# davidesantangelo/krep

Measured on NVIDIA H100. Metric: GB/s scanned (HBM-resident corpus), higher is better.
Workload: dtype u8

## Files before the change

### include/krep_b200.h

```cpp
#ifndef KREP_B200_H
#define KREP_B200_H

#include <stdbool.h>
#include <stddef.h>
#include <stdint.h>

#ifdef __cplusplus
extern "C" {
#endif

#ifndef KREP_H

typedef struct
{
   size_t start_offset;
   size_t end_offset;
} match_position_t;

typedef struct match_result_t
{
   match_position_t *positions;
   uint64_t count;
   uint64_t capacity;
} match_result_t;

struct ac_trie;
typedef struct ac_trie ac_trie_t;

typedef struct search_params
{
   const char *pattern;
   size_t pattern_len;

   const char **patterns;
   size_t *pattern_lens;
   size_t num_patterns;

   bool case_sensitive;
   bool use_regex;
   bool count_lines_mode;
   bool count_matches_mode;
   bool track_positions;
   bool whole_word;

   const void *compiled_regex;
   ac_trie_t *ac_trie;
   size_t max_count;
} search_params_t;

typedef uint64_t (*search_func_t)(const search_params_t *params,
                                  const char *text_start,
                                  size_t text_len,
                                  match_result_t *result);
#endif


int krep_b200_init(int device);
int krep_b200_device_count(void);
void krep_b200_warmup(void);
void krep_b200_set_devices(const int *devices, int n);
void krep_b200_shutdown(void);
int krep_b200_last_error(void);
const char *krep_b200_last_error_string(void);
const char *krep_b200_version(void);

void krep_b200_set_only_matching(bool on);
bool krep_b200_get_only_matching(void);
void krep_b200_set_force_no_simd(bool on);
void krep_b200_set_algo_override(const char *name);

uint64_t krep_b200_boyer_moore_search(const search_params_t *, const char *, size_t, match_result_t *);
uint64_t krep_b200_kmp_search(const search_params_t *, const char *, size_t, match_result_t *);
uint64_t krep_b200_memchr_search(const search_params_t *, const char *, size_t, match_result_t *);
uint64_t krep_b200_memchr_short_search(const search_params_t *, const char *, size_t, match_result_t *);
uint64_t krep_b200_simd_sse42_search(const search_params_t *, const char *, size_t, match_result_t *);
uint64_t krep_b200_simd_avx2_search(const search_params_t *, const char *, size_t, match_result_t *);
uint64_t krep_b200_simd_avx512_search(const search_params_t *, const char *, size_t, match_result_t *);
uint64_t krep_b200_aho_corasick_search(const search_params_t *, const char *, size_t, match_result_t *);
uint64_t krep_b200_neon_search(const search_params_t *, const char *, size_t, match_result_t *);
uint64_t krep_b200_regex_search(const search_params_t *, const char *, size_t, match_result_t *);

int krep_b200_search_batch(search_func_t entry, const search_params_t *params, const char *const *texts,
                           const size_t *lens, size_t n_texts, uint64_t *counts, match_result_t *const *results);

search_func_t krep_b200_select_search_algorithm(const search_params_t *params);
const char *krep_b200_get_algorithm_name(search_func_t func);

ac_trie_t *krep_b200_ac_trie_build(const search_params_t *params);
void krep_b200_ac_trie_free(ac_trie_t *trie);
bool krep_b200_ac_trie_root_has_outputs(const ac_trie_t *trie);

match_result_t *krep_b200_match_result_init(uint64_t initial_capacity);
bool krep_b200_match_result_add(match_result_t *result, size_t start_offset, size_t end_offset);
void krep_b200_match_result_free(match_result_t *result);
bool krep_b200_match_result_merge(match_result_t *dest, const match_result_t *src, size_t chunk_offset);


enum
{
   KREP_B200_ALGO_BMH = 0,
   KREP_B200_ALGO_KMP = 1,
   KREP_B200_ALGO_MEMCHR = 2,
   KREP_B200_ALGO_MEMCHR_SHORT = 3,
   KREP_B200_ALGO_SSE42 = 4,
   KREP_B200_ALGO_AVX2 = 5,
   KREP_B200_ALGO_AVX512 = 6,
   KREP_B200_ALGO_AC = 7,
   KREP_B200_ALGO_NEON = 8,
   KREP_B200_ALGO_REGEX = 9
};

typedef struct krep_b200_plan krep_b200_plan_t;

krep_b200_plan_t *krep_b200_plan_create(const search_params_t *params, int algo);
void krep_b200_plan_destroy(krep_b200_plan_t *plan);
const char *krep_b200_plan_filter_name(const krep_b200_plan_t *plan);

typedef struct
{
   const void *d_text;
   uint64_t avail_len;
   uint64_t own_begin;
   uint64_t own_end;
   uint64_t global_offset;
   int32_t prev_byte;
   int32_t next_byte;
} krep_b200_shard_t;

typedef struct
{
   uint64_t count;
   uint64_t stored;
   const uint64_t *d_keys;
   int overflow;
   uint64_t text_len;
   const uint64_t *d_line_bounds;
   int32_t device;
   int32_t slot;
   uint64_t serial;
} krep_b200_device_result_t;

int krep_b200_scan_shard(const krep_b200_plan_t *plan, const krep_b200_shard_t *shard,
                         int want_positions, void *stream, krep_b200_device_result_t *out);
int krep_b200_scan_shard_begin(const krep_b200_plan_t *plan, const krep_b200_shard_t *shard,
                               int want_positions, void *stream, int *ticket);
int krep_b200_scan_shard_end(int ticket, krep_b200_device_result_t *out);

int krep_b200_export_keys(const krep_b200_device_result_t *dev, void *d_dst, uint64_t max_keys, void *stream);
int krep_b200_export_packed(const krep_b200_device_result_t *dev, void *d_dst, uint64_t max_keys, void *stream);
int krep_b200_export_packed_async(int ticket, void *d_dst, uint64_t max_keys);
uint64_t krep_b200_merge_keys(const uint64_t *const *lists, const uint64_t *counts, uint32_t n_lists, uint64_t *dst);

float krep_b200_last_kernel_ms(void);
uint64_t krep_b200_launch_count(void);
void krep_b200_reset_launch_count(void);

typedef struct
{
   uint64_t lines;
   uint32_t flags;
   uint32_t reserved;
} krep_b200_line_count_t;
enum
{
   KREP_B200_LINES_HAS_HIT = 1,
   KREP_B200_LINES_FIRST_OPEN = 2,
   KREP_B200_LINES_LAST_PENDING = 4,
   KREP_B200_LINES_HAS_NL = 8
};
int krep_b200_count_lines_shard(const krep_b200_plan_t *plan, const search_params_t *params, const krep_b200_shard_t *shard,
                                void *stream, krep_b200_line_count_t *out);
uint64_t krep_b200_combine_line_counts(const krep_b200_line_count_t *recs, size_t n, size_t max_count);

uint64_t krep_b200_collect(const krep_b200_plan_t *plan, const search_params_t *params,
                           const krep_b200_device_result_t *dev, match_result_t *result);

uint64_t krep_b200_search_shards(const krep_b200_plan_t *plan, const search_params_t *params,
                                 const krep_b200_shard_t *shards, uint32_t n_shards, match_result_t *result);

uint64_t krep_b200_replay(int algo, const search_params_t *params, bool only_matching,
                          const uint64_t *keys, uint64_t nkeys,
                          const char *text, size_t text_len, match_result_t *result);

int64_t krep_b200_regex_filter_host(const search_params_t *params, const char *text, size_t n, uint64_t *line_starts,
                                    uint64_t cap, int *widened);

int krep_b200_regex_count_mode(const search_params_t *params);
int64_t krep_b200_regex_count_host(const search_params_t *params, const char *text, size_t n, uint64_t reach);
int krep_b200_regex_match_mode(const search_params_t *params);
int64_t krep_b200_regex_matches_host(const search_params_t *params, const char *text, size_t n, uint64_t reach,
                                     match_result_t *res);
int64_t krep_b200_regex_scan_shard_raw(const krep_b200_plan_t *plan, const krep_b200_shard_t *shard, int mode,
                                       uint64_t *keys, uint64_t cap, uint64_t *device_lines);

uint64_t krep_b200_replay_lines(int algo, const search_params_t *params, bool only_matching,
                                const uint64_t *keys, uint64_t nkeys, const uint64_t *bounds,
                                size_t text_len, match_result_t *result);

uint64_t krep_b200_ac_key_end(uint64_t key);
uint64_t krep_b200_ac_key_start(uint64_t key);
uint32_t krep_b200_ac_key_pattern(uint64_t key);

typedef struct
{
   uint64_t seed;
   uint64_t plant_seed;
   uint64_t plant_period;
   const char *needle;
   uint32_t needle_len;
   uint32_t flags;
} krep_b200_corpus_spec_t;

enum
{
   KREP_B200_CORPUS_RANDOM_CASE = 1,
   KREP_B200_CORPUS_EMBED_HALF = 2
};

int krep_b200_corpus_generate(const krep_b200_corpus_spec_t *spec, void *d_dst,
                              uint64_t global_offset, uint64_t len, void *stream);
int krep_b200_corpus_generate_host(const krep_b200_corpus_spec_t *spec, void *dst,
                                   uint64_t global_offset, uint64_t len);

#ifdef __cplusplus
}
#endif
#endif
```

### krep_b200/csrc/engine.h

```cpp
#pragma once
#include <mutex>
#include <vector>
#include "common.h"

namespace kb {

static constexpr uint32_t PACK_KEYS = 16384;
static constexpr int SCAN_SLOTS = 2;

struct StageSlot
{
    uint8_t *buf = nullptr;
    cudaEvent_t ev = nullptr;
    bool in_flight = false;
};

struct PendingScan
{
    bool active = false;
    const Plan *plan = nullptr;
    krep_b200_shard_t shard;
    int want_positions = 0;
    cudaStream_t stream = nullptr;
};

struct DevCtx
{
    bool ready = false;
    int device = 0, sm_count = 0;
    cudaStream_t scan_stream = nullptr, copy_stream = nullptr;
    cudaStream_t fin_stream = nullptr;
    unsigned long long *d_counter = nullptr;
    bool counter_clean[SCAN_SLOTS] = {false, false};
    uint64_t *d_list[SCAN_SLOTS] = {nullptr, nullptr};
    uint64_t *d_alt = nullptr;
    uint64_t key_cap = 0;
    void *d_sort_tmp = nullptr;
    size_t sort_tmp_bytes = 0;
    uint64_t *d_bounds = nullptr;
    uint64_t bounds_cap = 0;
    uint64_t *h_bounds = nullptr;
    uint64_t h_bounds_cap = 0;
    uint64_t *d_pack[SCAN_SLOTS] = {nullptr, nullptr}, *h_pack[SCAN_SLOTS] = {nullptr, nullptr};
    cudaEvent_t ev_a[SCAN_SLOTS] = {nullptr, nullptr}, ev_b[SCAN_SLOTS] = {nullptr, nullptr};
    cudaEvent_t ev_done[SCAN_SLOTS] = {nullptr, nullptr};
    cudaEvent_t ev_scanned[SCAN_SLOTS] = {nullptr, nullptr};
    cudaEvent_t ev_ca = nullptr, ev_cb = nullptr;
    PendingScan pend[SCAN_SLOTS];
    int next_slot = 0;
    uint64_t serial = 0;
    cudaStream_t result_stream = nullptr;
    void *d_line_recs = nullptr;
    uint64_t line_recs_cap = 0;
    uint64_t *d_line_out = nullptr, *h_line_out = nullptr;
    uint64_t line_out_cap = 0;
    uint8_t *d_ring = nullptr;
    size_t ring_slot_bytes = 0;
    int ring_slots = 0;
    std::vector<cudaEvent_t> ring_landed, ring_scanned;
    std::vector<StageSlot> stage;
    size_t stage_bytes = 0;
    std::vector<cudaEvent_t> ev_pool;
    uint64_t *h_keys = nullptr;
    uint64_t h_keys_cap = 0;
    uint8_t *h_batch = nullptr;
    uint64_t h_batch_cap = 0;
};

struct ErrState
{
    int code = 0;
    char msg[512] = "";
};
void get_error(ErrState *e);
void adopt_error(const ErrState &e);

std::recursive_mutex &engine_mutex();
int primary_device();
int visible_devices();
DevCtx *ctx_get(int device);
DevCtx *ctx_primary();
void engine_shutdown();
void prewarm_host_path(DevCtx &C);
void keep_devices_visible();
void warm_join();
bool warm_running();

struct DeviceGuard
{
    int saved = -1;
    DeviceGuard() { if (cudaGetDevice(&saved) != cudaSuccess) { saved = -1; cudaGetLastError(); } }
    ~DeviceGuard() { if (saved >= 0) cudaSetDevice(saved); }
};

Plan *plan_build(const search_params_t *P, int algo, bool only_matching);
Plan *regex_plan_build(const search_params_t *P, std::string *why);
void plan_free(Plan *p);
const PlanDev *plan_on_device(const Plan *p, DevCtx &C);
int resolve_algo(const search_params_t *P, int algo);

unsigned long long *slot_counter(DevCtx &C, int slot);
int scan_begin(DevCtx &C, const Plan *plan, const krep_b200_shard_t *sh, int want_positions, cudaStream_t stream, int *slot);
int scan_end(DevCtx &C, int slot, ScanOut *out);
int scan_shard(DevCtx &C, const Plan *plan, const krep_b200_shard_t *sh, int want_positions, cudaStream_t stream, ScanOut *out);
int finish_scan(DevCtx &C, int slot, int want_sort, cudaStream_t stream);
int ensure_keys(DevCtx &C, uint64_t cap);
int reset_counter(DevCtx &C, int slot, cudaStream_t stream);
int sort_keys(DevCtx &C, int slot, uint64_t n, int end_bit, cudaStream_t stream, const uint64_t **sorted);
int key_end_bit(const Plan *plan, uint64_t max_offset, bool regex_matches = false);
int fetch_keys(DevCtx &C, const ScanOut &so, const uint64_t **h);
void add_kernel_ms(float ms);
void reset_kernel_ms();
float get_kernel_ms();
void set_kernel_ms(float ms);
void trace(const char *fmt, ...);

bool count_lines_eligible(const Plan *plan, const search_params_t *P, int algo);
int ensure_line_out(DevCtx &C, uint64_t n);
int launch_count_lines(DevCtx &C, const Plan *plan, const krep_b200_shard_t *sh, cudaStream_t stream, uint64_t index);
uint64_t combine_line_records(const uint64_t *recs, size_t n);

uint64_t merge_key_lists(const uint64_t *const *lists, const uint64_t *counts, uint32_t n_lists, uint64_t *dst);

}
```

### krep_b200/csrc/host_api.cu

```cuda
#include <algorithm>
#include <cstdio>
#include <cstdlib>
#include <cstring>
#include <omp.h>
#include <sys/mman.h>
#include <thread>
#include "common.h"
#include "engine.h"

namespace kb {

static bool g_only_matching = false;
static bool g_force_no_simd = false;
static std::string g_algo_override;

static constexpr size_t SIMD_MAX_PATTERN_LEN = 32;

int resolve_algo(const search_params_t *P, int algo)
{
    const size_t m = P->pattern_len;
    if (algo == KREP_B200_ALGO_AVX512)
    {
        if (m == 0 || m > 64 || !P->case_sensitive) return KREP_B200_ALGO_BMH;
        if (m <= 32) algo = KREP_B200_ALGO_AVX2;
    }
    if (algo == KREP_B200_ALGO_AVX2)
    {
        if (m == 0 || m > 32 || !P->case_sensitive) return KREP_B200_ALGO_BMH;
        if (m <= 16) algo = KREP_B200_ALGO_SSE42;
    }
    if (algo == KREP_B200_ALGO_SSE42)
    {
        if (m == 0 || m > 16 || !P->case_sensitive) return KREP_B200_ALGO_BMH;
    }
    if (algo == KREP_B200_ALGO_NEON && (m == 0 || !P->case_sensitive)) return KREP_B200_ALGO_BMH;
    return algo;
}

static std::vector<Plan *> g_plan_cache;

static bool plan_matches(const Plan *pl, const search_params_t *P, int algo, bool only_matching)
{
    if (pl->is_regex || algo == KREP_B200_ALGO_REGEX) return false;
    if (pl->algo != algo || pl->case_sensitive != P->case_sensitive || pl->count_lines != P->count_lines_mode) return false;
    if (pl->is_ac)
    {
        if ((pl->whole_word != 0) != P->whole_word) return false;
        if (pl->patterns.size() != P->num_patterns) return false;
        for (size_t k = 0; k < P->num_patterns; k++)
        {
            if (pl->pat_lens[k] != P->pattern_lens[k]) return false;
            if (P->pattern_lens[k] && memcmp(pl->patterns[k].data(), P->patterns[k], P->pattern_lens[k]) != 0) return false;
        }
        return true;
    }
    size_t m = algo == KREP_B200_ALGO_MEMCHR ? (P->pattern_len ? 1 : 0) : P->pattern_len;
    if (pl->m != m || memcmp(pl->pattern.data(), P->pattern, m) != 0) return false;
    if ((pl->whole_word != 0) != P->whole_word) return false;
    return pl->built_only_matching == only_matching;
}

static void cache_insert(Plan *pl)
{
    if (g_plan_cache.size() >= 16)
    {
        plan_free(g_plan_cache.front());
        g_plan_cache.erase(g_plan_cache.begin());
    }
    g_plan_cache.push_back(pl);
}

static Plan *cached_plan(const search_params_t *P, int algo, bool only_matching)
{
    for (size_t i = 0; i < g_plan_cache.size(); i++)
        if (plan_matches(g_plan_cache[i], P, algo, only_matching))
        {
            Plan *pl = g_plan_cache[i];
            g_plan_cache.erase(g_plan_cache.begin() + i);
            g_plan_cache.push_back(pl);
            return pl;
        }
    Plan *pl = plan_build(P, algo, only_matching);
    if (pl) cache_insert(pl);
    return pl;
}

static Plan *cached_regex_plan(const search_params_t *P, std::string *why)
{
    std::string re;
    if (!regex_source(P, &re))
    {
        *why = "no pattern";
        return nullptr;
    }
    for (size_t i = 0; i < g_plan_cache.size(); i++)
    {
        Plan *pl = g_plan_cache[i];
        if (pl->is_regex && pl->regex == re && pl->case_sensitive == P->case_sensitive)
        {
            g_plan_cache.erase(g_plan_cache.begin() + i);
            g_plan_cache.push_back(pl);
            return pl;
        }
    }
    Plan *pl = regex_plan_build(P, why);
    if (pl) cache_insert(pl);
    return pl;
}

void plan_cache_clear()
{
    for (Plan *p : g_plan_cache) plan_free(p);
    g_plan_cache.clear();
}

struct TrieHandle
{
    uint64_t magic;
    Plan *plan;
};
static constexpr uint64_t TRIE_MAGIC = 0x6b7265705f747269ull;

#define CKH(call)                                                                                  \
    do                                                                                             \
    {                                                                                              \
        cudaError_t e_ = (call);                                                                   \
        if (e_ != cudaSuccess)                                                                     \
        {                                                                                          \
            set_error(-2, "CUDA error %s at %s:%d (%s)", cudaGetErrorName(e_), __FILE__, __LINE__, \
                      cudaGetErrorString(e_));                                                     \
            return -2;                                                                             \
        }                                                                                          \
    } while (0)

static size_t env_mb(const char *name, size_t dflt_mb)
{
    const char *v = getenv(name);
    if (!v || !*v) return dflt_mb << 20;
    long x = atol(v);
    return x > 0 ? (size_t)x << 20 : dflt_mb << 20;
}

static int ensure_ring(DevCtx &E, size_t slot_bytes, int slots)
{
    slot_bytes = (slot_bytes + 255) & ~(size_t)255;
    if (E.ring_slot_bytes >= slot_bytes && E.ring_slots >= slots) return 0;
    CKH(cudaDeviceSynchronize());
    cudaFree(E.d_ring);
    E.d_ring = nullptr;
    E.ring_slot_bytes = 0;
    E.ring_slots = 0;
    cudaError_t e = cudaMalloc(&E.d_ring, slot_bytes * slots);
    if (e != cudaSuccess)
    {
        set_error(-2, "cannot allocate %zu bytes of HBM for the staging ring (%s)", slot_bytes * slots, cudaGetErrorString(e));
        return -2;
    }
    E.ring_slot_bytes = slot_bytes;
    E.ring_slots = slots;
    while ((int)E.ring_landed.size() < slots)
    {
        cudaEvent_t a, b;
        CKH(cudaEventCreateWithFlags(&a, cudaEventDisableTiming));
        CKH(cudaEventCreateWithFlags(&b, cudaEventDisableTiming));
        E.ring_landed.push_back(a);
        E.ring_scanned.push_back(b);
    }
    return 0;
}

static int ensure_stage(DevCtx &E, size_t bytes, int slots)
{
    if (E.stage_bytes >= bytes && (int)E.stage.size() >= slots) return 0;
    for (auto &s : E.stage)
    {
        cudaFreeHost(s.buf);
        if (s.ev) cudaEventDestroy(s.ev);
    }
    E.stage.clear();
    E.stage.resize(slots);
    for (auto &s : E.stage)
    {
        CKH(cudaMallocHost(&s.buf, bytes));
        CKH(cudaEventCreateWithFlags(&s.ev, cudaEventDisableTiming));
        s.in_flight = false;
    }
    E.stage_bytes = bytes;
    return 0;
}

static cudaEvent_t pool_event(DevCtx &E, size_t idx)
{
    while (E.ev_pool.size() <= idx)
    {
        cudaEvent_t ev;
        cudaEventCreate(&ev);
        E.ev_pool.push_back(ev);
    }
    return E.ev_pool[idx];
}

static int copy_threads()
{
    static int nt = 0;
    if (!nt)
    {
        const char *v = getenv("KREP_B200_COPY_THREADS");
        nt = v ? atoi(v) : 8;
        nt = std::max(1, std::min(nt, std::max(1, omp_get_num_procs())));
    }
    return nt;
}

static inline void populate_piece(const uint8_t *src, size_t n)
{
#ifndef MADV_POPULATE_READ
#define MADV_POPULATE_READ 22
#endif
    static const bool on = !getenv("KREP_B200_NO_POPULATE_READ");
    if (!on) return;
    const uintptr_t a = (uintptr_t)src & ~(uintptr_t)4095, e = ((uintptr_t)src + n + 4095) & ~(uintptr_t)4095;
    (void)madvise((void *)a, e - a, MADV_POPULATE_READ);
}

static void parallel_copy(uint8_t *dst, const uint8_t *src, size_t n)
{
    const int nt = copy_threads();
    if (n < (8u << 20) || nt == 1)
    {
        populate_piece(src, n);
        memcpy(dst, src, n);
        return;
    }
    const size_t piece = (n / nt + 4095) & ~(size_t)4095;
#pragma omp parallel for num_threads(nt) schedule(static)
    for (int i = 0; i < nt; i++)
    {
        const size_t off = (size_t)i * piece;
        if (off < n)
        {
            populate_piece(src + off, std::min(piece, n - off));
            memcpy(dst + off, src + off, std::min(piece, n - off));
        }
    }
}

static bool is_pinned(const void *p)
{
    cudaPointerAttributes a;
    if (cudaPointerGetAttributes(&a, p) != cudaSuccess)
    {
        cudaGetLastError();
        return false;
    }
    return a.type == cudaMemoryTypeHost;
}

void prewarm_host_path(DevCtx &E)
{
    const size_t slot = env_mb("KREP_B200_STAGE_MB", 32) + 4096;
    if (ensure_ring(E, slot, 3) != 0 || ensure_stage(E, slot, 3) != 0 || ensure_keys(E, 1) != 0) clear_error();
}

struct RangeJob
{
    DevCtx *C = nullptr;
    const Plan *plan = nullptr;
    const char *text = nullptr;
    size_t n = 0, begin = 0, end = 0, chunk = 0;
    int want_positions = 0;
    bool pinned = false;
    bool count_lines = false;
    std::vector<uint64_t> line_recs;
    bool regex_count = false;
    uint64_t regex_lines = 0;
    bool regex_matches = false;
    int rc = 0;
    ScanOut so;
    const uint64_t *h_keys = nullptr;
    std::vector<uint64_t> own_keys;
    float kernel_ms = 0.f;
    ErrState err;
};

static int stream_range(RangeJob &J)
{
    DevCtx &E = *J.C;
    CKH(cudaSetDevice(E.device));
    const Plan *plan = J.plan;
    if (!plan_on_device(plan, E)) return -2;
    const uint32_t halo = plan->is_regex ? REGEX_HALO : (plan->is_ac ? plan->max_len : plan->m) + 1;
    const size_t chunk = J.chunk, n = J.n;
    const size_t span = J.end - J.begin;
    const size_t nchunks = (span + chunk - 1) / chunk;
    const int nslots = nchunks >= 3 ? 3 : (int)std::max<size_t>(nchunks, 1);
    if (ensure_ring(E, std::min(chunk, span) + halo + 64, nslots) != 0) return -2;
    if (!J.pinned && ensure_stage(E, std::min(chunk, span) + halo + 64, nslots) != 0) return -2;
    if (J.want_positions && ensure_keys(E, 1) != 0) return -2;
    if (J.count_lines && ensure_line_out(E, nchunks) != 0) return -2;
    if (J.regex_count && ensure_line_out(E, 1) != 0) return -2;
    unsigned long long *d_regex_lines = J.regex_count ? (unsigned long long *)E.d_line_out : nullptr;
    reset_kernel_ms();
    const int slot = 0;
    for (int attempt = 0; attempt < 3; attempt++)
    {
        CKH(cudaStreamWaitEvent(E.scan_stream, E.ev_done[slot], 0));
        if (reset_counter(E, slot, E.scan_stream) != 0) return -2;
        if (d_regex_lines) CKH(cudaMemsetAsync(d_regex_lines, 0, sizeof(unsigned long long), E.scan_stream));
        for (size_t c = 0; c < nchunks; c++)
        {
            const size_t off = J.begin + c * chunk, len = std::min(chunk, J.end - off);
            const size_t src_len = std::min(len + halo, n - off);
            const int rs = (int)(c % E.ring_slots);
            uint8_t *d_slot = E.d_ring + (size_t)rs * E.ring_slot_bytes;
            if (c >= (size_t)E.ring_slots) CKH(cudaStreamWaitEvent(E.copy_stream, E.ring_scanned[rs], 0));
            if (J.pinned)
                CKH(cudaMemcpyAsync(d_slot, J.text + off, src_len, cudaMemcpyHostToDevice, E.copy_stream));
            else
            {
                StageSlot &s = E.stage[c % E.stage.size()];
                if (s.in_flight) CKH(cudaEventSynchronize(s.ev));
                parallel_copy(s.buf, (const uint8_t *)J.text + off, src_len);
                CKH(cudaMemcpyAsync(d_slot, s.buf, src_len, cudaMemcpyHostToDevice, E.copy_stream));
                CKH(cudaEventRecord(s.ev, E.copy_stream));
                s.in_flight = true;
            }
            CKH(cudaEventRecord(E.ring_landed[rs], E.copy_stream));
            CKH(cudaStreamWaitEvent(E.scan_stream, E.ring_landed[rs], 0));
            krep_b200_shard_t part;
            part.d_text = d_slot;
            part.avail_len = src_len;
            part.own_begin = 0;
            part.own_end = len;
            part.global_offset = off;
            part.prev_byte = off > 0 ? (int32_t)(uint8_t)J.text[off - 1] : -1;
            part.next_byte = off + src_len < n ? (int32_t)(uint8_t)J.text[off + src_len] : -1;
            cudaEvent_t a = pool_event(E, 2 * c), b = pool_event(E, 2 * c + 1);
            CKH(cudaEventRecord(a, E.scan_stream));
            int rc = J.count_lines ? launch_count_lines(E, plan, &part, E.scan_stream, c)
                                   : launch_scan(E, plan, &part, J.want_positions, E.scan_stream, slot, d_regex_lines,
                                                 J.regex_matches);
            if (rc != 0) return rc;
            CKH(cudaEventRecord(b, E.scan_stream));
            CKH(cudaEventRecord(E.ring_scanned[rs], E.scan_stream));
        }
        CKH(cudaGetLastError());
        if (!J.count_lines && finish_scan(E, slot, J.want_positions, E.scan_stream) != 0) return -2;
        if (d_regex_lines) CKH(cudaMemcpyAsync(E.h_line_out, d_regex_lines, sizeof(uint64_t), cudaMemcpyDeviceToHost, E.scan_stream));
        CKH(cudaStreamSynchronize(E.scan_stream));
        if (!J.count_lines) CKH(cudaEventSynchronize(E.ev_done[slot]));
        for (auto &s : E.stage) s.in_flight = false;
        for (size_t c = 0; c < nchunks; c++)
        {
            float ms = 0.f;
            if (cudaEventElapsedTime(&ms, E.ev_pool[2 * c], E.ev_pool[2 * c + 1]) == cudaSuccess) add_kernel_ms(ms);
            else cudaGetLastError();
        }
        if (J.count_lines)
        {
            J.line_recs.assign(E.h_line_out, E.h_line_out + 2 * nchunks);
            J.so = ScanOut();
            return 0;
        }
        if (J.regex_count) J.regex_lines = E.h_line_out[0];
        const uint64_t cnt = E.h_pack[slot][0];
        J.so = ScanOut();
        J.so.count = cnt;
        J.so.device = E.device;
        J.so.serial = ++E.serial;
        E.result_stream = E.scan_stream;
        if (!J.want_positions) return 0;
        if (cnt <= E.key_cap)
        {
            J.so.stored = cnt;
            if (cnt <= PACK_KEYS)
            {
                J.so.d_keys = E.d_pack[slot] + 1;
                J.so.h_sorted = E.h_pack[slot] + 1;
                return 0;
            }
            return sort_keys(E, slot, cnt, key_end_bit(plan, n, J.regex_matches), E.scan_stream, &J.so.d_keys);
        }
        J.so.overflow = 1;
        if (ensure_keys(E, cnt + cnt / 8 + 1024) != 0) return -2;
        reset_kernel_ms();
    }
    set_error(-4, "occurrence list kept overflowing");
    return -4;
}

static std::vector<int> g_devices;

static std::vector<int> host_devices(size_t n)
{
    std::vector<int> out;
    const int vis = visible_devices();
    if (vis == 0) return out;
    if (!g_devices.empty())
    {
        for (int d : g_devices)
            if (d >= 0 && d < vis && std::find(out.begin(), out.end(), d) == out.end()) out.push_back(d);
        if (!out.empty()) return out;
    }
    const int prim = primary_device();
    if (prim < 0) return out;
    int want = 1;
    const char *v = getenv("KREP_B200_DEVICES");
    if (v && *v && atoi(v) > 0) want = atoi(v);
    want = std::max(1, std::min(want, vis));
    out.push_back(prim);
    for (int d = 0; d < vis && (int)out.size() < want; d++)
        if (d != prim) out.push_back(d);
    return out;
}

struct HostScan
{
    uint64_t count = 0;
    const uint64_t *keys = nullptr;
    uint64_t nkeys = 0;
    std::vector<uint64_t> merged;
    uint64_t regex_lines = 0;
};

static int stage_and_scan(const Plan *plan, const char *text, size_t n, int want_positions, HostScan *hs, bool count_lines = false,
                          bool regex_matches = false)
{
    const bool pinned = is_pinned(text);
    const size_t chunk = pinned ? env_mb("KREP_B200_CHUNK_MB", 256) : env_mb("KREP_B200_STAGE_MB", 32);
    std::vector<int> devs = host_devices(n);
    if (devs.empty())
    {
        set_error(-1, "no CUDA device available; this engine has no CPU fallback");
        return -1;
    }
    const size_t nchunks = std::max<size_t>((n + chunk - 1) / chunk, 1);
    if (devs.size() > nchunks) devs.resize(nchunks);
    const size_t D = devs.size();
    size_t R = D;
    if (const char *v = getenv("KREP_B200_RANGES"))
        if (atoi(v) > 0) R = std::min<size_t>(std::max<size_t>((size_t)atoi(v), D), nchunks);
    std::vector<RangeJob> jobs(R);
    const size_t per = (nchunks + R - 1) / R;
    for (size_t i = 0; i < R; i++)
    {
        RangeJob &J = jobs[i];
        J.plan = plan;
        J.text = text;
        J.n = n;
        J.chunk = chunk;
        J.begin = std::min(i * per * chunk, n);
        J.end = std::min((i + 1) * per * chunk, n);
        J.want_positions = want_positions;
        J.pinned = pinned;
        J.count_lines = count_lines && !plan->is_regex;
        J.regex_count = count_lines && plan->is_regex;
        J.regex_matches = regex_matches;
    }
    trace("search: %zu bytes (%s host memory), %zu device(s), %zu range(s), chunk %zu MiB", n, pinned ? "pinned" : "pageable", D, R,
          chunk >> 20);
    auto run_device = [&jobs, &devs, D, R](size_t d) {
        for (size_t i = d; i < R; i += D)
        {
            RangeJob &J = jobs[i];
            J.C = ctx_get(devs[d]);
            if (!J.C)
            {
                J.rc = -1;
                break;
            }
            J.rc = J.begin < J.end ? stream_range(J) : 0;
            J.kernel_ms = get_kernel_ms();
            if (J.rc != 0) break;
            if (R > D && J.so.stored)
            {
                const uint64_t *k = nullptr;
                if ((J.rc = fetch_keys(*J.C, J.so, &k)) != 0) break;
                J.own_keys.assign(k, k + J.so.stored);
                J.h_keys = J.own_keys.data();
            }
        }
    };
    if (D == 1)
    {
        run_device(0);
        float ksum = 0.f;
        for (auto &J : jobs)
        {
            if (J.rc != 0) return J.rc;
            ksum += J.kernel_ms;
        }
        set_kernel_ms(ksum);
    }
    else
    {
        std::vector<std::thread> th;
        for (size_t d = 0; d < D; d++)
            th.emplace_back([&jobs, &run_device, d, D, R] {
                clear_error();
                run_device(d);
                for (size_t i = d; i < R; i += D) get_error(&jobs[i].err);
            });
        for (auto &t : th) t.join();
        std::vector<float> kdev(D, 0.f);
        for (size_t i = 0; i < R; i++)
        {
            if (jobs[i].rc != 0)
            {
                adopt_error(jobs[i].err);
                return jobs[i].rc;
            }
            kdev[i % D] += jobs[i].kernel_ms;
        }
        set_kernel_ms(*std::max_element(kdev.begin(), kdev.end()));
    }
    trace("search: all ranges scanned (slowest device: %.2f ms of scan kernels)", get_kernel_ms());
    hs->count = 0;
    hs->keys = nullptr;
    hs->nkeys = 0;
    hs->regex_lines = 0;
    if (count_lines && !plan->is_regex)
    {
        std::vector<uint64_t> all;
        for (auto &J : jobs) all.insert(all.end(), J.line_recs.begin(), J.line_recs.end());
        hs->count = combine_line_records(all.data(), all.size() / 2);
        return 0;
    }
    for (auto &J : jobs)
    {
        hs->count += J.so.count;
        hs->regex_lines += J.regex_lines;
    }
    if (!want_positions) return 0;
    for (auto &J : jobs)
    {
        if (J.so.stored == 0 || J.h_keys || !J.C) continue;
        cudaSetDevice(J.C->device);
        if (fetch_keys(*J.C, J.so, &J.h_keys) != 0) return -2;
    }
    if (R == 1)
    {
        hs->keys = jobs[0].h_keys;
        hs->nkeys = jobs[0].so.stored;
        return 0;
    }
    std::vector<const uint64_t *> lists;
    std::vector<uint64_t> counts;
    uint64_t total = 0;
    for (auto &J : jobs)
    {
        lists.push_back(J.h_keys);
        counts.push_back(J.so.stored);
        total += J.so.stored;
    }
    hs->merged.resize(total);
    hs->nkeys = merge_key_lists(lists.data(), counts.data(), (uint32_t)lists.size(), hs->merged.data());
    hs->keys = hs->merged.data();
    trace("search: merged %llu keys from %zu ranges", (unsigned long long)hs->nkeys, R);
    return 0;
}

static bool keeps_all(int algo, bool only_matching, const search_params_t *P, const Plan *pl)
{
    if (pl->is_ac) return true;
    if (pl->emit_len != pl->m) return false;
    if (algo == KREP_B200_ALGO_AVX2 || algo == KREP_B200_ALGO_AVX512 || algo == KREP_B200_ALGO_NEON) return false;
    if (pl->border_free) return true;
    switch (algo)
    {
    case KREP_B200_ALGO_BMH: return !(only_matching && !P->count_lines_mode);
    case KREP_B200_ALGO_MEMCHR: return true;
    case KREP_B200_ALGO_MEMCHR_SHORT: return !only_matching;
    case KREP_B200_ALGO_SSE42: return only_matching;
    default: return false;
    }
}

static uint64_t limited_count(int algo, const search_params_t *P, uint64_t total)
{
    const uint64_t maxc = P->max_count;
    switch (algo)
    {
    case KREP_B200_ALGO_BMH:
    case KREP_B200_ALGO_MEMCHR_SHORT:
        if (total == 0) return 0;
        return maxc == 0 ? 1 : std::min<uint64_t>(total, maxc);
    default:
        return std::min<uint64_t>(total, maxc);
    }
}

static bool early_answer(int entry_algo, const search_params_t *P, const char *text, size_t n, match_result_t *res, int *algo_out,
                         uint64_t *ret)
{
    *ret = 0;
    int algo = entry_algo;
    size_t m = 0;
    if (algo == KREP_B200_ALGO_AC)
    {
        if (!P->ac_trie || !text) return true;
        if (P->max_count == 0) return true;
        if (n == 0)
        {
            for (size_t k = 0; k < P->num_patterns; k++)
                if (P->pattern_lens[k] == 0)
                {
                    if (P->track_positions && res) result_push(res, 0, 0);
                    *ret = 1;
                    return true;
                }
            return true;
        }
    }
    else
    {
        algo = resolve_algo(P, algo);
        m = P->pattern_len;
        switch (algo)
        {
        case KREP_B200_ALGO_KMP:
            if (P->max_count == 0) return true;
            if (m == 0 || n < m) return true;
            break;
        case KREP_B200_ALGO_MEMCHR:
            if (P->max_count == 0 || n == 0) return true;
            m = 1;
            break;
        case KREP_B200_ALGO_MEMCHR_SHORT:
            if (P->max_count == 0 && (P->count_lines_mode || P->track_positions)) return true;
            if (m < 2 || m > 3 || n < m) return true;
            break;
        default:
            if (P->max_count == 0 && (P->count_lines_mode || P->track_positions)) return true;
            if (m == 0 || n < m) return true;
            break;
        }
        if (!P->pattern) return true;
        if (m > 1024)
        {
            set_error(-3, "pattern longer than 1024 bytes (MAX_PATTERN_LENGTH, krep.c:77)");
            return true;
        }
    }
    *algo_out = algo;
    return false;
}

static Plan *plan_for(const search_params_t *P, int algo, bool only_matching)
{
    if (algo == KREP_B200_ALGO_AC && P->ac_trie)
    {
        const TrieHandle *h = reinterpret_cast<const TrieHandle *>(P->ac_trie);
        if (h->magic == TRIE_MAGIC && h->plan && plan_matches(h->plan, P, algo, only_matching)) return h->plan;
    }
    return cached_plan(P, algo, only_matching);
}

static uint64_t run_search(int entry_algo, const search_params_t *P, const char *text, size_t n, match_result_t *res)
{
    std::lock_guard<std::recursive_mutex> lk(engine_mutex());
    clear_error();
    if (!P) return 0;
    const bool only_matching = g_only_matching;
    int algo = entry_algo;
    uint64_t early = 0;
    if (early_answer(entry_algo, P, text, n, res, &algo, &early)) return early;
    if (warm_running())
    {
        if (n >= (64u << 20) && getenv("KREP_B200_PREFAULT"))
        {
            trace("search: pre-faulting %zu bytes while the context comes up", n);
            const long pages = (long)((n + 4095) / 4096);
            unsigned long sink = 0;
#pragma omp parallel for num_threads(copy_threads()) schedule(static) reduction(+ : sink)
            for (long pg = 0; pg < pages; pg++) sink += (unsigned char)text[(size_t)pg * 4096];
            if (sink == 0x5EED5EED5EEDull) trace("(unlikely checksum)");
        }
        warm_join();
        trace("search: context ready");
    }
    if (visible_devices() == 0)
    {
        set_error(-1, "no CUDA device available; this engine has no CPU fallback");
        return 0;
    }
    DeviceGuard guard;
    Plan *plan = plan_for(P, algo, only_matching);
    if (!plan) return 0;
    const bool want_result = P->track_positions && res;
    const bool need_list = P->count_lines_mode || want_result || !keeps_all(algo, only_matching, P, plan) ||
                           plan->whole_word == 2;
    HostScan hs;
    if (count_lines_eligible(plan, P, algo) && !getenv("KREP_B200_NO_FUSED_COUNT"))
    {
        if (stage_and_scan(plan, text, n, 0, &hs, true) != 0) return 0;
        return std::min<uint64_t>(hs.count, P->max_count);
    }
    if (stage_and_scan(plan, text, n, need_list ? 1 : 0, &hs) != 0) return 0;
    if (!need_list) return limited_count(algo, P, hs.count);
    Replay r{hs.keys, (size_t)hs.nkeys, text, n, 0};
    const uint64_t ret = plan->is_ac ? replay_ac(P, r, res) : replay_literal(algo, P, only_matching, plan->m, r, res);
    trace("search: replay done (%llu)", (unsigned long long)ret);
    return ret;
}

static bool regex_count_exact(const search_params_t *P, const Plan *plan)
{
    return P->count_lines_mode && !P->whole_word && plan->rx->count_exact;
}

static bool regex_count_fused(const search_params_t *P, const Plan *plan)
{
    return regex_count_exact(P, plan) && !getenv("KREP_B200_NO_FUSED_COUNT");
}

static uint64_t regex_count_total(const search_params_t *P, uint64_t device_lines, const Replay &uncertain)
{
    return std::min<uint64_t>(device_lines + replay_regex(P, uncertain, nullptr), P->max_count);
}

static bool regex_matches_exact(const search_params_t *P, const Plan *plan)
{
    return P->track_positions && !P->count_lines_mode && !P->whole_word && plan->rx->offsets_exact;
}

static bool regex_matches_device(const search_params_t *P, const Plan *plan)
{
    return regex_matches_exact(P, plan) && !getenv("KREP_B200_NO_DEVICE_MATCHES");
}

static uint64_t run_regex(const search_params_t *P, const char *text, size_t n, match_result_t *res)
{
    std::lock_guard<std::recursive_mutex> lk(engine_mutex());
    clear_error();
    if (!P) return 0;
    if (P->max_count == 0 && (P->count_lines_mode || P->track_positions)) return 0;
    if (!P->compiled_regex) return 0;
    Replay r{nullptr, 0, text, n, 0};
    if (n == 0) return replay_regex(P, r, res);
    if (!text) return 0;
    warm_join();
    if (visible_devices() == 0)
    {
        set_error(-1, "no CUDA device available; this engine has no CPU fallback");
        return 0;
    }
    DeviceGuard guard;
    std::string why;
    Plan *plan = cached_regex_plan(P, &why);
    if (!plan)
    {
        set_error(-3, "this regex is not run on the GPU (%s); krep_b200_select_search_algorithm returns NULL for it", why.c_str());
        return 0;
    }
    const bool fused = regex_count_fused(P, plan);
    const bool matches = !fused && regex_matches_device(P, plan);
    HostScan hs;
    if (stage_and_scan(plan, text, n, 1, &hs, fused, matches) != 0) return 0;
    r.keys = hs.keys;
    r.n = (size_t)hs.nkeys;
    if (matches)
    {
        const uint64_t ret = replay_regex_matches(P, r, res);
        trace("search: regex offsets on the device: %llu keys (%llu)", (unsigned long long)hs.nkeys, (unsigned long long)ret);
        return ret;
    }
    if (fused)
    {
        const uint64_t ret = regex_count_total(P, hs.regex_lines, r);
        trace("search: regex -c fused: %llu lines counted on the device, %llu uncertain lines to regexec (%llu)",
              (unsigned long long)hs.regex_lines, (unsigned long long)hs.nkeys, (unsigned long long)ret);
        return ret;
    }
    const uint64_t ret = replay_regex(P, r, res);
    trace("search: regex confirmed on %llu flagged lines (%llu)", (unsigned long long)hs.nkeys, (unsigned long long)ret);
    return ret;
}

static int run_batch(int entry_algo, const search_params_t *P, const char *const *texts, const size_t *lens, size_t nt,
                     uint64_t *counts, match_result_t *const *results)
{
    warm_join();
    std::lock_guard<std::recursive_mutex> lk(engine_mutex());
    clear_error();
    if (!P || !texts || !lens || !counts)
    {
        set_error(-3, "krep_b200_search_batch: null argument");
        return -3;
    }
    const bool only_matching = g_only_matching;
    std::vector<int> algo_of(nt, -1);
    int algo = -1;
    for (size_t f = 0; f < nt; f++)
    {
        int a = entry_algo;
        uint64_t early = 0;
        counts[f] = 0;
        if (early_answer(entry_algo, P, texts[f], lens[f], results ? results[f] : nullptr, &a, &early)) counts[f] = early;
        else algo_of[f] = algo = a;
    }
    if (krep_b200_last_error() != 0) return -3;
    if (algo < 0) return 0;
    DeviceGuard guard;
    DevCtx *Cp = ctx_primary();
    if (!Cp) return -1;
    Plan *plan = plan_for(P, algo, only_matching);
    if (!plan) return -2;
    const size_t gap = (size_t)(plan->is_ac ? plan->max_len : plan->m) + 16;
    std::vector<uint64_t> off(nt, 0);
    uint64_t total = 0;
    for (size_t f = 0; f < nt; f++)
        if (algo_of[f] >= 0)
        {
            off[f] = total;
            total = (total + lens[f] + gap + 15) & ~15ull;
        }
    DevCtx &E = *Cp;
    if (total > E.h_batch_cap)
    {
        cudaFreeHost(E.h_batch);
        E.h_batch = nullptr;
        E.h_batch_cap = 0;
        CKH(cudaMallocHost(&E.h_batch, total + total / 4 + 4096));
        E.h_batch_cap = total + total / 4 + 4096;
    }
    {
        std::vector<size_t> live;
        for (size_t f = 0; f < nt; f++)
            if (algo_of[f] >= 0) live.push_back(f);
        const long nl = (long)live.size();
        uint8_t *const hb = E.h_batch;
#pragma omp parallel for num_threads(copy_threads()) schedule(dynamic, 16)
        for (long i = 0; i < nl; i++)
        {
            const size_t f = live[(size_t)i];
            const uint64_t end = off[f] + lens[f], next = i + 1 < nl ? off[live[(size_t)i + 1]] : total;
            memcpy(hb + off[f], texts[f], lens[f]);
            memset(hb + end, 0, next - end);
        }
    }
    HostScan hs;
    if (stage_and_scan(plan, (const char *)E.h_batch, total, 1, &hs) != 0) return -2;
    const uint64_t *keys = hs.keys;
    struct { uint64_t stored; } so{hs.nkeys};
    std::vector<uint64_t> mine;
    size_t j = 0;
    for (size_t f = 0; f < nt; f++)
    {
        if (algo_of[f] < 0) continue;
        const uint64_t lo = off[f], hi = off[f] + lens[f];
        mine.clear();
        auto span = [&](uint64_t key, uint64_t *s, uint64_t *e) {
            if (plan->is_ac)
            {
                *e = key >> AC_END_SHIFT;
                *s = *e - (1024 - ((key >> AC_LEN_SHIFT) & 1023));
            }
            else
            {
                *s = key >> LIT_TAG_BITS;
                *e = *s + ((key >> 2) & 1 ? plan->m : plan->emit_len);
            }
        };
        while (j < so.stored)
        {
            uint64_t s, e;
            span(keys[j], &s, &e);
            const uint64_t ord = plan->is_ac ? e : s;
            if (ord >= hi + (plan->is_ac ? gap : 0)) break;
            if (s >= lo && e <= hi) mine.push_back(keys[j]);
            j++;
        }
        Replay r{mine.data(), mine.size(), texts[f], lens[f], lo};
        match_result_t *res = results ? results[f] : nullptr;
        counts[f] = plan->is_ac ? replay_ac(P, r, res) : replay_literal(algo, P, only_matching, plan->m, r, res);
    }
    return 0;
}

}

using namespace kb;

extern "C" {

void krep_b200_set_only_matching(bool on) { g_only_matching = on; }
bool krep_b200_get_only_matching(void) { return g_only_matching; }
void krep_b200_set_force_no_simd(bool on) { g_force_no_simd = on; }
void krep_b200_set_algo_override(const char *name) { g_algo_override = name ? name : ""; }

uint64_t krep_b200_boyer_moore_search(const search_params_t *p, const char *t, size_t n, match_result_t *r)
{
    return run_search(KREP_B200_ALGO_BMH, p, t, n, r);
}
uint64_t krep_b200_kmp_search(const search_params_t *p, const char *t, size_t n, match_result_t *r)
{
    return run_search(KREP_B200_ALGO_KMP, p, t, n, r);
}
uint64_t krep_b200_memchr_search(const search_params_t *p, const char *t, size_t n, match_result_t *r)
{
    return run_search(KREP_B200_ALGO_MEMCHR, p, t, n, r);
}
uint64_t krep_b200_memchr_short_search(const search_params_t *p, const char *t, size_t n, match_result_t *r)
{
    return run_search(KREP_B200_ALGO_MEMCHR_SHORT, p, t, n, r);
}
uint64_t krep_b200_simd_sse42_search(const search_params_t *p, const char *t, size_t n, match_result_t *r)
{
    return run_search(KREP_B200_ALGO_SSE42, p, t, n, r);
}
uint64_t krep_b200_simd_avx2_search(const search_params_t *p, const char *t, size_t n, match_result_t *r)
{
    return run_search(KREP_B200_ALGO_AVX2, p, t, n, r);
}
uint64_t krep_b200_simd_avx512_search(const search_params_t *p, const char *t, size_t n, match_result_t *r)
{
    return run_search(KREP_B200_ALGO_AVX512, p, t, n, r);
}
uint64_t krep_b200_aho_corasick_search(const search_params_t *p, const char *t, size_t n, match_result_t *r)
{
    return run_search(KREP_B200_ALGO_AC, p, t, n, r);
}
uint64_t krep_b200_neon_search(const search_params_t *p, const char *t, size_t n, match_result_t *r)
{
    return run_search(KREP_B200_ALGO_NEON, p, t, n, r);
}
uint64_t krep_b200_regex_search(const search_params_t *p, const char *t, size_t n, match_result_t *r)
{
    return run_regex(p, t, n, r);
}

int krep_b200_search_batch(search_func_t entry, const search_params_t *params, const char *const *texts, const size_t *lens,
                           size_t n_texts, uint64_t *counts, match_result_t *const *results)
{
    int algo = -1;
    if (entry == krep_b200_boyer_moore_search) algo = KREP_B200_ALGO_BMH;
    else if (entry == krep_b200_kmp_search) algo = KREP_B200_ALGO_KMP;
    else if (entry == krep_b200_memchr_search) algo = KREP_B200_ALGO_MEMCHR;
    else if (entry == krep_b200_memchr_short_search) algo = KREP_B200_ALGO_MEMCHR_SHORT;
    else if (entry == krep_b200_simd_sse42_search) algo = KREP_B200_ALGO_SSE42;
    else if (entry == krep_b200_simd_avx2_search) algo = KREP_B200_ALGO_AVX2;
    else if (entry == krep_b200_simd_avx512_search) algo = KREP_B200_ALGO_AVX512;
    else if (entry == krep_b200_aho_corasick_search) algo = KREP_B200_ALGO_AC;
    else if (entry == krep_b200_neon_search) algo = KREP_B200_ALGO_NEON;
    if (entry == krep_b200_regex_search)
    {
        set_error(-3, "krep_b200_search_batch: regex searches are not batched; call krep_b200_regex_search per text");
        return -3;
    }
    if (algo < 0)
    {
        set_error(-3, "krep_b200_search_batch: entry must be one of this library's search_func_t entry points");
        return -3;
    }
    return run_batch(algo, params, texts, lens, n_texts, counts, results);
}

static bool is_repetitive_pattern(const char *pattern, size_t len)
{
    if (len < 3) return false;
    size_t run = 0;
    char prev = pattern[0];
    for (size_t i = 1; i < len; i++)
    {
        if (pattern[i] == prev)
        {
            if (++run >= len / 2) return true;
        }
        else
        {
            run = 0;
            prev = pattern[i];
        }
    }
    for (size_t period = 2; period <= len / 2; period++)
    {
        bool periodic = true;
        for (size_t i = period; i < len && periodic; i++) periodic = pattern[i] == pattern[i % period];
        if (periodic) return true;
    }
    return false;
}

search_func_t krep_b200_select_search_algorithm(const search_params_t *P)
{
    if (!P) return NULL;
    if (P->use_regex)
    {
        std::lock_guard<std::recursive_mutex> lk(engine_mutex());
        std::string why;
        return cached_regex_plan(P, &why) ? krep_b200_regex_search : NULL;
    }
    if (P->num_patterns > 1) return krep_b200_aho_corasick_search;
    if (!g_algo_override.empty() && g_algo_override != "auto")
    {
        if (g_algo_override == "bm") return krep_b200_boyer_moore_search;
        if (g_algo_override == "kmp") return krep_b200_kmp_search;
    }
    const size_t m = P->pattern_len;
    const bool can_simd = !g_force_no_simd && m <= SIMD_MAX_PATTERN_LEN;
    if (m == 1) return krep_b200_memchr_search;
    if (m < 4) return (can_simd && P->case_sensitive) ? krep_b200_simd_avx2_search : krep_b200_memchr_short_search;
    if (can_simd && m <= 32) return krep_b200_simd_avx2_search;
    if (m < 8 && is_repetitive_pattern(P->pattern, m)) return krep_b200_kmp_search;
    return krep_b200_boyer_moore_search;
}

const char *krep_b200_get_algorithm_name(search_func_t f)
{
    if (f == krep_b200_boyer_moore_search) return "Boyer-Moore-Horspool";
    if (f == krep_b200_kmp_search) return "Knuth-Morris-Pratt";
    if (f == krep_b200_aho_corasick_search) return "Aho-Corasick";
    if (f == krep_b200_memchr_search) return "memchr";
    if (f == krep_b200_memchr_short_search) return "memchr-short";
    if (f == krep_b200_simd_sse42_search) return "SSE4.2";
    if (f == krep_b200_simd_avx2_search) return "AVX2";
    if (f == krep_b200_simd_avx512_search) return "AVX-512";
    if (f == krep_b200_neon_search) return "NEON";
    if (f == krep_b200_regex_search) return "Regex (GPU line filter + regexec)";
    return "Unknown";
}

ac_trie_t *krep_b200_ac_trie_build(const search_params_t *params)
{
    warm_join();
    std::lock_guard<std::recursive_mutex> lk(engine_mutex());
    clear_error();
    if (!params || params->num_patterns == 0) return NULL;
    if (visible_devices() == 0)
    {
        set_error(-1, "no CUDA device available; this engine has no CPU fallback");
        return NULL;
    }
    Plan *pl = plan_build(params, KREP_B200_ALGO_AC, false);
    if (!pl) return NULL;
    TrieHandle *h = new TrieHandle{TRIE_MAGIC, pl};
    return reinterpret_cast<ac_trie_t *>(h);
}
void krep_b200_ac_trie_free(ac_trie_t *trie)
{
    TrieHandle *h = reinterpret_cast<TrieHandle *>(trie);
    if (!h || h->magic != TRIE_MAGIC) return;
    std::lock_guard<std::recursive_mutex> lk(engine_mutex());
    plan_free(h->plan);
    h->magic = 0;
    delete h;
}
bool krep_b200_ac_trie_root_has_outputs(const ac_trie_t *trie)
{
    const TrieHandle *h = reinterpret_cast<const TrieHandle *>(trie);
    if (!h || h->magic != TRIE_MAGIC || !h->plan) return false;
    for (uint32_t len : h->plan->pat_lens)
        if (len == 0) return true;
    return false;
}

void krep_b200_set_devices(const int *devices, int n)
{
    std::lock_guard<std::recursive_mutex> lk(engine_mutex());
    if (devices && n > 0) keep_devices_visible();
    g_devices.clear();
    for (int i = 0; devices && i < n; i++) g_devices.push_back(devices[i]);
}

match_result_t *krep_b200_match_result_init(uint64_t initial_capacity)
{
    match_result_t *r = (match_result_t *)malloc(sizeof *r);
    if (!r) return NULL;
    if (initial_capacity == 0) initial_capacity = 16;
    if (initial_capacity > SIZE_MAX / sizeof(match_position_t))
    {
        free(r);
        return NULL;
    }
    r->positions = (match_position_t *)malloc(initial_capacity * sizeof(match_position_t));
    if (!r->positions)
    {
        free(r);
        return NULL;
    }
    r->count = 0;
    r->capacity = initial_capacity;
    return r;
}
bool krep_b200_match_result_add(match_result_t *r, size_t s, size_t e) { return result_push(r, s, e); }
void krep_b200_match_result_free(match_result_t *r)
{
    if (!r) return;
    free(r->positions);
    free(r);
}
bool krep_b200_match_result_merge(match_result_t *dest, const match_result_t *src, size_t chunk_offset)
{
    if (!dest || !src || src->count == 0) return true;
    for (uint64_t i = 0; i < src->count; i++)
        if (!result_push(dest, src->positions[i].start_offset + chunk_offset, src->positions[i].end_offset + chunk_offset))
            return false;
    return true;
}

uint64_t krep_b200_replay(int algo, const search_params_t *P, bool only_matching, const uint64_t *keys, uint64_t nkeys,
                          const char *text, size_t text_len, match_result_t *result)
{
    if (!P) return 0;
    if (P->count_lines_mode && !text && nkeys)
    {
        set_error(-3, "krep_b200_replay: -c line counting needs the host text");
        return 0;
    }
    if (algo == KREP_B200_ALGO_REGEX)
    {
        clear_error();
        if (!text && text_len)
        {
            set_error(-3, "krep_b200_replay: regex keys are confirmed by regexec on the host text");
            return 0;
        }
        return replay_regex(P, Replay{keys, (size_t)nkeys, text, text_len, 0}, result);
    }
    Replay r{keys, (size_t)nkeys, text, text_len ? text_len : (SIZE_MAX >> 1), 0};
    if (algo == KREP_B200_ALGO_AC) return replay_ac(P, r, result);
    algo = resolve_algo(P, algo);
    const uint32_t m = algo == KREP_B200_ALGO_MEMCHR ? 1u : (uint32_t)P->pattern_len;
    return replay_literal(algo, P, only_matching, m, r, result);
}

uint64_t krep_b200_replay_lines(int algo, const search_params_t *P, bool only_matching, const uint64_t *keys, uint64_t nkeys,
                                const uint64_t *bounds, size_t text_len, match_result_t *result)
{
    if (!P) return 0;
    if (algo == KREP_B200_ALGO_REGEX)
    {
        set_error(-3, "krep_b200_replay_lines: regex keys need the host text (krep_b200_replay)");
        return 0;
    }
    if (P->count_lines_mode && !bounds && nkeys)
    {
        set_error(-3, "krep_b200_replay_lines: -c needs the line bounds");
        return 0;
    }
    Replay r{keys, (size_t)nkeys, nullptr, text_len ? text_len : (SIZE_MAX >> 1), 0, bounds};
    if (algo == KREP_B200_ALGO_AC) return replay_ac(P, r, result);
    algo = resolve_algo(P, algo);
    const uint32_t m = algo == KREP_B200_ALGO_MEMCHR ? 1u : (uint32_t)P->pattern_len;
    return replay_literal(algo, P, only_matching, m, r, result);
}

int krep_b200_count_lines_shard(const krep_b200_plan_t *plan_, const search_params_t *P, const krep_b200_shard_t *shard, void *stream,
                                krep_b200_line_count_t *out)
{
    std::lock_guard<std::recursive_mutex> lk(engine_mutex());
    clear_error();
    const Plan *plan = reinterpret_cast<const Plan *>(plan_);
    if (!plan || !P || !shard || !out)
    {
        set_error(-3, "krep_b200_count_lines_shard: null argument");
        return -3;
    }
    if (!count_lines_eligible(plan, P, plan->algo))
    {
        set_error(-3, "krep_b200_count_lines_shard: this plan's -c result needs the occurrence list (pattern set, window kernel, "
                      "newline in the pattern or tag-mode -w): use krep_b200_scan_shard + krep_b200_collect");
        return -3;
    }
    DeviceGuard guard;
    cudaPointerAttributes a;
    DevCtx *C = (cudaPointerGetAttributes(&a, shard->d_text) == cudaSuccess && a.type == cudaMemoryTypeDevice) ? ctx_get(a.device) : ctx_primary();
    if (!C) return -1;
    cudaStream_t st = stream ? (cudaStream_t)stream : C->scan_stream;
    reset_kernel_ms();
    if (cudaEventRecord(C->ev_ca, st) != cudaSuccess) return -2;
    int rc = launch_count_lines(*C, plan, shard, st, 0);
    if (rc != 0) return rc;
    if (cudaEventRecord(C->ev_cb, st) != cudaSuccess || cudaStreamSynchronize(st) != cudaSuccess)
    {
        set_error(-2, "CUDA error in the fused line count (%s)", cudaGetErrorString(cudaGetLastError()));
        return -2;
    }
    float ms = 0.f;
    cudaEventElapsedTime(&ms, C->ev_ca, C->ev_cb);
    add_kernel_ms(ms);
    out->lines = C->h_line_out[0];
    out->flags = (uint32_t)C->h_line_out[1];
    out->reserved = 0;
    return 0;
}

uint64_t krep_b200_combine_line_counts(const krep_b200_line_count_t *recs, size_t n, size_t max_count)
{
    if (!recs) return 0;
    std::vector<uint64_t> flat(2 * n);
    for (size_t i = 0; i < n; i++)
    {
        flat[2 * i] = recs[i].lines;
        flat[2 * i + 1] = recs[i].flags;
    }
    return std::min<uint64_t>(combine_line_records(flat.data(), n), max_count);
}

uint64_t krep_b200_search_shards(const krep_b200_plan_t *plan_, const search_params_t *P, const krep_b200_shard_t *shards,
                                 uint32_t n_shards, match_result_t *result)
{
    std::lock_guard<std::recursive_mutex> lk(engine_mutex());
    clear_error();
    const Plan *plan = reinterpret_cast<const Plan *>(plan_);
    if (!plan || !P || (!shards && n_shards))
    {
        set_error(-3, "krep_b200_search_shards: null argument");
        return 0;
    }
    if (plan->is_regex)
    {
        set_error(-3, "krep_b200_search_shards: regex plans need the host text: scan the shards, merge the keys and call "
                      "krep_b200_replay with KREP_B200_ALGO_REGEX");
        return 0;
    }
    DeviceGuard guard;
    std::vector<DevCtx *> ctx(n_shards, nullptr);
    uint64_t text_len = 0;
    for (uint32_t i = 0; i < n_shards; i++)
    {
        cudaPointerAttributes a;
        ctx[i] = (cudaPointerGetAttributes(&a, shards[i].d_text) == cudaSuccess && a.type == cudaMemoryTypeDevice) ? ctx_get(a.device)
                                                                                                                    : ctx_primary();
        if (!ctx[i]) return 0;
        text_len = std::max<uint64_t>(text_len, shards[i].global_offset + shards[i].avail_len);
    }
    reset_kernel_ms();
    if (P->count_lines_mode)
    {
        if (!count_lines_eligible(plan, P, plan->algo))
        {
            set_error(-3, "krep_b200_search_shards: -c over several shards is only available where the scan counts lines itself "
                          "(single literals; see krep_b200_count_lines_shard)");
            return 0;
        }
        if (P->max_count == 0) return 0;
        std::vector<uint64_t> recs(2 * (size_t)n_shards);
        for (uint32_t i = 0; i < n_shards; i++)
        {
            cudaSetDevice(ctx[i]->device);
            if (ensure_line_out(*ctx[i], n_shards) != 0) return 0;
        }
        for (uint32_t i = 0; i < n_shards; i++)
        {
            cudaSetDevice(ctx[i]->device);
            if (launch_count_lines(*ctx[i], plan, &shards[i], ctx[i]->scan_stream, i) != 0) return 0;
        }
        for (uint32_t i = 0; i < n_shards; i++)
        {
            cudaSetDevice(ctx[i]->device);
            if (cudaStreamSynchronize(ctx[i]->scan_stream) != cudaSuccess)
            {
                set_error(-2, "CUDA error in the fused line count (%s)", cudaGetErrorString(cudaGetLastError()));
                return 0;
            }
            recs[2 * i] = ctx[i]->h_line_out[2 * i];
            recs[2 * i + 1] = ctx[i]->h_line_out[2 * i + 1];
        }
        return std::min<uint64_t>(combine_line_records(recs.data(), n_shards), P->max_count);
    }
    const bool need_list = (P->track_positions && result) || !keeps_all(plan->algo, plan->built_only_matching, P, plan) || plan->whole_word == 2;
    std::vector<std::vector<uint64_t>> keys(n_shards);
    std::vector<int> pending(MAX_DEV, -1);
    std::vector<int> slot_of(n_shards, 0);
    uint64_t total_count = 0;
    float kmax = 0.f;
    auto finish = [&](int i) -> int {
        DevCtx &C = *ctx[i];
        cudaSetDevice(C.device);
        ScanOut so;
        int rc = scan_end(C, slot_of[i], &so);
        kmax = std::max(kmax, get_kernel_ms());
        if (rc != 0) return rc;
        total_count += so.count;
        if (need_list && so.stored)
        {
            const uint64_t *k = nullptr;
            if ((rc = fetch_keys(C, so, &k)) != 0) return rc;
            keys[i].assign(k, k + so.stored);
        }
        return 0;
    };
    for (uint32_t i = 0; i < n_shards; i++)
    {
        DevCtx &C = *ctx[i];
        if (pending[C.device] >= 0)
        {
            if (finish(pending[C.device]) != 0) return 0;
            pending[C.device] = -1;
        }
        cudaSetDevice(C.device);
        if (scan_begin(C, plan, &shards[i], need_list ? 1 : 0, nullptr, &slot_of[i]) != 0) return 0;
        pending[C.device] = (int)i;
    }
    for (int d = 0; d < MAX_DEV; d++)
        if (pending[d] >= 0 && finish(pending[d]) != 0) return 0;
    set_kernel_ms(kmax);
    if (!need_list) return limited_count(plan->algo, P, total_count);
    std::vector<const uint64_t *> lists;
    std::vector<uint64_t> counts;
    uint64_t total = 0;
    for (auto &k : keys)
    {
        lists.push_back(k.data());
        counts.push_back(k.size());
        total += k.size();
    }
    std::vector<uint64_t> merged(total ? total : 1);
    const uint64_t nk = merge_key_lists(lists.data(), counts.data(), (uint32_t)lists.size(), merged.data());
    Replay r{merged.data(), (size_t)nk, nullptr, text_len ? (size_t)text_len : (SIZE_MAX >> 1), 0};
    if (plan->is_ac) return replay_ac(P, r, result);
    return replay_literal(plan->algo, P, plan->built_only_matching, plan->m, r, result);
}

uint64_t krep_b200_collect(const krep_b200_plan_t *plan_, const search_params_t *P, const krep_b200_device_result_t *dev,
                           match_result_t *result)
{
    std::lock_guard<std::recursive_mutex> lk(engine_mutex());
    clear_error();
    const Plan *plan = reinterpret_cast<const Plan *>(plan_);
    if (!plan || !P || !dev) return 0;
    if (plan->is_regex)
    {
        set_error(-3, "krep_b200_collect: regex plans need the host text: export the keys and call krep_b200_replay with "
                      "KREP_B200_ALGO_REGEX");
        return 0;
    }
    if (P->count_lines_mode && dev->stored && !dev->d_line_bounds)
    {
        set_error(-3, "krep_b200_collect: -c needs a plan created with count_lines_mode (line bounds are computed by the scan)");
        return 0;
    }
    if (!dev->stored) return limited_count(plan->algo, P, plan->is_ac || keeps_all(plan->algo, g_only_matching, P, plan) ? dev->count : 0);
    DeviceGuard guard;
    DevCtx *Cp = ctx_get(dev->device);
    if (!Cp) return 0;
    DevCtx &E = *Cp;
    ScanOut so;
    so.count = dev->count;
    so.stored = dev->stored;
    so.d_keys = dev->d_keys;
    if (dev->serial == E.serial && dev->stored <= PACK_KEYS && dev->slot >= 0 && dev->slot < SCAN_SLOTS)
        so.h_sorted = E.h_pack[dev->slot] + 1;
    const uint64_t *keys = nullptr;
    if (fetch_keys(E, so, &keys) != 0) return 0;
    Replay r{keys, (size_t)so.stored, nullptr, dev->text_len ? (size_t)dev->text_len : (SIZE_MAX >> 1), 0};
    if (P->count_lines_mode)
    {
        const uint64_t nb = 2 * so.stored;
        if (nb > E.h_bounds_cap)
        {
            cudaFreeHost(E.h_bounds);
            E.h_bounds = nullptr;
            E.h_bounds_cap = 0;
            if (cudaMallocHost(&E.h_bounds, (nb + nb / 4 + 1024) * sizeof(uint64_t)) != cudaSuccess)
            {
                set_error(-2, "cannot allocate pinned memory for line bounds");
                return 0;
            }
            E.h_bounds_cap = nb + nb / 4 + 1024;
        }
        cudaStream_t st = E.result_stream ? E.result_stream : E.scan_stream;
        if (cudaMemcpyAsync(E.h_bounds, dev->d_line_bounds, nb * sizeof(uint64_t), cudaMemcpyDeviceToHost, st) != cudaSuccess ||
            cudaStreamSynchronize(st) != cudaSuccess)
        {
            set_error(-2, "reading line bounds back failed");
            return 0;
        }
        uint64_t *b = E.h_bounds;
        for (uint64_t i = 0; i < so.stored; i++)
            if (b[2 * i] == LB_SAME_AS_PREV) b[2 * i] = i ? b[2 * (i - 1)] : LB_OUTSIDE_SHARD;
        for (uint64_t i = so.stored; i-- > 0;)
            if (b[2 * i + 1] == LB_SAME_AS_NEXT) b[2 * i + 1] = i + 1 < so.stored ? b[2 * (i + 1) + 1] : LB_OUTSIDE_SHARD;
        for (uint64_t i = 0; i < nb; i++)
            if (b[i] == LB_OUTSIDE_SHARD)
            {
                set_error(-3, "krep_b200_collect: a matching line continues into a neighbouring shard; -c needs newline-aligned shards");
                return 0;
            }
        r.bounds = b;
    }
    if (plan->is_ac) return replay_ac(P, r, result);
    return replay_literal(plan->algo, P, plan->built_only_matching, plan->m, r, result);
}

int64_t krep_b200_regex_filter_host(const search_params_t *P, const char *text, size_t n, uint64_t *line_starts, uint64_t cap,
                                    int *widened)
{
    std::lock_guard<std::recursive_mutex> lk(engine_mutex());
    std::string why;
    Plan *pl = P ? cached_regex_plan(P, &why) : nullptr;
    if (!pl) return -1;
    std::vector<uint64_t> v;
    regex_lines_host(*pl->rx, text, text ? n : 0, &v);
    for (size_t i = 0; i < v.size() && i < cap; i++) line_starts[i] = v[i];
    if (widened) *widened = pl->rx->widened ? 1 : 0;
    return (int64_t)v.size();
}

int krep_b200_regex_count_mode(const search_params_t *P)
{
    std::lock_guard<std::recursive_mutex> lk(engine_mutex());
    std::string why;
    Plan *pl = P ? cached_regex_plan(P, &why) : nullptr;
    if (!pl) return -1;
    return regex_count_fused(P, pl) ? 1 : 0;
}

int64_t krep_b200_regex_count_host(const search_params_t *P, const char *text, size_t n, uint64_t reach)
{
    std::lock_guard<std::recursive_mutex> lk(engine_mutex());
    std::string why;
    Plan *pl = P ? cached_regex_plan(P, &why) : nullptr;
    if (!pl || !regex_count_exact(P, pl)) return -1;
    if (P->max_count == 0 || !P->compiled_regex) return 0;
    if (n == 0) return (int64_t)replay_regex(P, Replay{nullptr, 0, text, 0, 0}, nullptr);
    if (!text) return 0;
    std::vector<uint64_t> keys;
    const uint64_t device_lines = regex_count_lines_host(*pl->rx, text, n, reach, &keys);
    for (uint64_t &k : keys) k <<= LIT_TAG_BITS;
    return (int64_t)regex_count_total(P, device_lines, Replay{keys.data(), keys.size(), text, n, 0});
}

int krep_b200_regex_match_mode(const search_params_t *P)
{
    std::lock_guard<std::recursive_mutex> lk(engine_mutex());
    std::string why;
    Plan *pl = P ? cached_regex_plan(P, &why) : nullptr;
    if (!pl) return -1;
    return regex_matches_device(P, pl) ? 1 : 0;
}

int64_t krep_b200_regex_matches_host(const search_params_t *P, const char *text, size_t n, uint64_t reach, match_result_t *res)
{
    std::lock_guard<std::recursive_mutex> lk(engine_mutex());
    std::string why;
    Plan *pl = P ? cached_regex_plan(P, &why) : nullptr;
    if (!pl || !regex_matches_exact(P, pl)) return -1;
    if (P->max_count == 0 || !P->compiled_regex) return 0;
    if (n == 0) return (int64_t)replay_regex(P, Replay{nullptr, 0, text, 0, 0}, res);
    if (!text) return 0;
    std::vector<uint64_t> keys;
    regex_matches_host(*pl->rx, text, n, reach, &keys);
    return (int64_t)replay_regex_matches(P, Replay{keys.data(), keys.size(), text, n, 0}, res);
}

}
```

### krep_b200/csrc/lit_filters.cuh

```cuda
#pragma once
#include "common.h"

namespace kb {

__device__ __forceinline__ bool dev_is_word(int c)
{
    return (c >= '0' && c <= '9') || (c >= 'A' && c <= 'Z') || (c >= 'a' && c <= 'z') || c == '_';
}

__device__ __forceinline__ unsigned verify_exact(const LitDevParams &p, long long cand)
{
    if (cand < (long long)p.own_begin || cand >= (long long)p.own_end) return 0;
    const uint64_t c = (uint64_t)cand;
    if (c + p.emit_len > p.avail_len) return 0;
    const uint8_t *t = p.text + c;
    const uint8_t *val = p.pat_val, *msk = p.pat_mask;
    for (uint32_t k = 0; k < p.emit_len; k++)
        if ((t[k] & msk[k]) != val[k]) return 0;
    unsigned full = 1;
    if (p.m > p.emit_len)
    {
        if (c + p.m > p.avail_len) full = 0;
        else
            for (uint32_t k = p.emit_len; k < p.m; k++)
                if ((t[k] & msk[k]) != val[k]) { full = 0; break; }
    }
    unsigned ww_tag = 3;
    if (p.whole_word)
    {
        const uint64_t e = c + p.m;
        const int pb = c > 0 ? (int)t[-1] : p.prev_byte;
        const int nb = e < p.avail_len ? (int)p.text[e] : p.next_byte;
        ww_tag = (dev_is_word(pb) ? 0u : 2u) | (dev_is_word(nb) ? 0u : 1u);
        if (p.whole_word == 1 && ww_tag != 3) return 0;
    }
    return 8u | (full << 2) | ww_tag;
}

__device__ __forceinline__ uint4 ld_stream(const uint4 *ptr)
{
    return __ldcs(ptr);
}

template <bool FOLD>
__device__ __forceinline__ bool hit_word(uint32_t w, uint32_t fold, uint32_t k0, uint32_t k1, uint32_t k2, uint32_t k3)
{
    if (FOLD) w &= fold;
    return (w == k0) | (w == k1) | (w == k2) | (w == k3);
}
template <bool FOLD>
__device__ __forceinline__ bool hit_vec(const uint4 &v, uint32_t fold, uint32_t k0, uint32_t k1, uint32_t k2, uint32_t k3)
{
    return hit_word<FOLD>(v.x, fold, k0, k1, k2, k3) | hit_word<FOLD>(v.y, fold, k0, k1, k2, k3) |
           hit_word<FOLD>(v.z, fold, k0, k1, k2, k3) | hit_word<FOLD>(v.w, fold, k0, k1, k2, k3);
}

template <bool MASKED>
__device__ __forceinline__ bool hit_pair(uint32_t lo, uint32_t hi, uint32_t mask, uint32_t k0, uint32_t c1, uint32_t c2,
                                         uint32_t c3)
{
    uint32_t x0 = lo, x1 = hi * c1 + __umulhi(lo, c1), x2 = hi * c2 + __umulhi(lo, c2), x3 = hi * c3 + __umulhi(lo, c3);
    if (MASKED)
    {
        x0 &= mask; x1 &= mask; x2 &= mask; x3 &= mask;
    }
    return (x0 == k0) | (x1 == k0) | (x2 == k0) | (x3 == k0);
}
template <bool FOLD, bool MASKED>
__device__ __forceinline__ bool hit_vec_w(const uint4 &v, uint32_t nx, uint32_t fold, uint32_t mask, uint32_t k0,
                                          uint32_t c1, uint32_t c2, uint32_t c3)
{
    uint32_t w0 = v.x, w1 = v.y, w2 = v.z, w3 = v.w, w4 = nx;
    if (FOLD)
    {
        w0 &= fold; w1 &= fold; w2 &= fold; w3 &= fold; w4 &= fold;
    }
    return hit_pair<MASKED>(w0, w1, mask, k0, c1, c2, c3) | hit_pair<MASKED>(w1, w2, mask, k0, c1, c2, c3) |
           hit_pair<MASKED>(w2, w3, mask, k0, c1, c2, c3) | hit_pair<MASKED>(w3, w4, mask, k0, c1, c2, c3);
}


}
```

### krep_b200/csrc/scan_count.cu

```cuda
#include <algorithm>
#include "engine.h"
#include "lit_filters.cuh"

namespace kb {

enum : uint32_t
{
    LR_HAS_HIT = 1,
    LR_FIRST_OPEN = 2,
    LR_LAST_PENDING = 4,
    LR_HAS_NL = 8
};

struct LineRec
{
    uint32_t lines, flags;
};

struct CountDev
{
    LitDevParams p;
    uint64_t own_end;
    uint32_t part_groups, n_parts;
    uint32_t exact;
    uint32_t tail;
    LineRec *recs;
};

struct PartState
{
    uint32_t lines = 0;
    bool has_hit = false, first_open = false, pending = false, seen_nl = false;
    uint64_t covered_to = 0;
};

__device__ __noinline__ unsigned verify_exact_call(const LitDevParams &p, long long cand) { return verify_exact(p, cand); }

__device__ __forceinline__ uint32_t nl_nibble(uint32_t w)
{
    const uint32_t x = w ^ 0x0A0A0A0Au;
    const uint32_t y = ~(((x & 0x7F7F7F7Fu) + 0x7F7F7F7Fu) | x | 0x7F7F7F7Fu);
    return ((y >> 7) * 0x10204080u) >> 28;
}
__device__ __forceinline__ uint32_t nl_mask16(const uint4 &v)
{
    return nl_nibble(v.x) | (nl_nibble(v.y) << 4) | (nl_nibble(v.z) << 8) | (nl_nibble(v.w) << 12);
}
__device__ __forceinline__ uint32_t range_mask16(uint64_t unit, uint64_t lo, uint64_t hi)
{
    uint32_t m = 0xFFFFu;
    if (unit < lo) m = lo - unit >= 16 ? 0u : (m & ~((1u << (uint32_t)(lo - unit)) - 1u));
    if (unit + 16 > hi) m = hi <= unit ? 0u : (m & ((1u << (uint32_t)(hi - unit)) - 1u));
    return m;
}

__device__ __noinline__ bool scan_for_newline(const LitDevParams &p, uint64_t lo, uint64_t hi)
{
    const uint32_t lane = threadIdx.x & 31;
    if (hi > p.avail_len) hi = p.avail_len;
    for (uint64_t base = lo & ~15ull; base < hi; base += 512)
    {
        const uint64_t unit = base + 16ull * lane;
        uint32_t nm = 0;
        if (unit < hi && unit + 16 > lo)
        {
            if (unit + 16 <= p.avail_len) nm = nl_mask16(__ldg(reinterpret_cast<const uint4 *>(p.text + unit)));
            else
                for (uint64_t q = unit; q < p.avail_len; q++) nm |= (p.text[q] == '\n' ? 1u : 0u) << (uint32_t)(q - unit);
            nm &= range_mask16(unit, lo, hi);
        }
        if (__any_sync(0xffffffffu, nm != 0)) return true;
    }
    return false;
}

__device__ __forceinline__ void settle(const LitDevParams &p, PartState &S, uint64_t upto)
{
    if (S.covered_to < upto && (S.pending || (!S.has_hit && !S.seen_nl)))
        if (scan_for_newline(p, S.covered_to, upto))
        {
            S.pending = false;
            S.seen_nl = true;
        }
}

__device__ __forceinline__ void account(PartState &S, uint32_t hm, uint32_t nm)
{
    const uint32_t lane = threadIdx.x & 31;
    const bool has_nl = nm != 0;
    const uint32_t fnl = has_nl ? (uint32_t)__ffs(nm) - 1 : 0, lnl = has_nl ? 31u - (uint32_t)__clz(nm) : 0;
    const bool f = has_nl && (hm & ((1u << fnl) - 1u)) != 0;
    const bool l = has_nl && ((hm >> lnl) >> 1) != 0;
    uint32_t inner = 0;
    if (__popc(nm) >= 2)
    {
        uint32_t prev = fnl, rest = nm & (nm - 1);
        while (rest)
        {
            const uint32_t nx = (uint32_t)__ffs(rest) - 1;
            if (hm & (((1u << nx) - 1u) & ~((2u << prev) - 1u))) inner++;
            prev = nx;
            rest &= rest - 1;
        }
    }
    const uint32_t A = __ballot_sync(0xffffffffu, has_nl), T = __ballot_sync(0xffffffffu, !has_nl && hm != 0);
    const uint32_t F = __ballot_sync(0xffffffffu, f), Lm = __ballot_sync(0xffffffffu, l);
    uint32_t innersum = 0;
    if (__ballot_sync(0xffffffffu, inner != 0)) innersum = __reduce_add_sync(0xffffffffu, inner);
    if (A == 0)
    {
        if (T)
        {
            if (!S.pending)
            {
                S.lines++;
                if (!S.has_hit && !S.seen_nl) S.first_open = true;
            }
            S.pending = true;
            S.has_hit = true;
        }
        return;
    }
    const uint32_t j1 = (uint32_t)__ffs(A) - 1, jr = 31u - (uint32_t)__clz(A);
    if ((T & ((1u << j1) - 1u)) || ((F >> j1) & 1u))
    {
        if (!S.pending)
        {
            S.lines++;
            if (!S.has_hit && !S.seen_nl) S.first_open = true;
        }
        S.has_hit = true;
    }
    S.pending = false;
    S.seen_nl = true;
    bool gap = false;
    if (has_nl && lane != j1)
    {
        const uint32_t below = A & ((1u << lane) - 1u);
        const uint32_t pj = 31u - (uint32_t)__clz(below);
        const uint32_t between = ((1u << lane) - 1u) & ~((2u << pj) - 1u);
        gap = ((Lm >> pj) & 1u) || (T & between) || f;
    }
    const uint32_t G = __ballot_sync(0xffffffffu, gap);
    S.lines += (uint32_t)__popc(G) + innersum;
    if (G || innersum) S.has_hit = true;
    if (((Lm >> jr) & 1u) || ((T >> jr) >> 1))
    {
        S.lines++;
        S.has_hit = true;
        S.pending = true;
    }
}

__device__ __forceinline__ uint64_t pack_state(const PartState &S)
{
    return (uint64_t)S.lines | ((uint64_t)((S.has_hit ? 1u : 0u) | (S.first_open ? 2u : 0u) | (S.pending ? 4u : 0u) | (S.seen_nl ? 8u : 0u)) << 32);
}
__device__ __forceinline__ void unpack_state(uint64_t k, PartState &S)
{
    S.lines = (uint32_t)k;
    const uint32_t f = (uint32_t)(k >> 32);
    S.has_hit = f & 1u;
    S.first_open = f & 2u;
    S.pending = f & 4u;
    S.seen_nl = f & 8u;
}
__device__ __noinline__ uint64_t account_call(uint64_t packed, uint32_t hm, uint32_t nm)
{
    PartState S;
    unpack_state(packed, S);
    account(S, hm, nm);
    return pack_state(S);
}

template <bool WINDOW>
__device__ __noinline__ uint32_t hit_mask16(const CountDev &D, uint64_t unit, const uint4 &v, uint32_t nx)
{
    const LitDevParams &p = D.p;
    const uint32_t w[5] = {v.x, v.y, v.z, v.w, nx};
    uint32_t hm = 0;
    if (WINDOW)
    {
        const uint32_t mask = p.fold & p.win_mask, k0 = p.K[0];
#pragma unroll
        for (int k = 0; k < 4; k++)
#pragma unroll
            for (int r = 0; r < 4; r++)
            {
                const uint32_t win = r == 0 ? w[k] : __funnelshift_r(w[k], w[k + 1], 8 * r);
                if ((win & mask) == k0)
                {
                    const uint64_t st = unit + 4 * k + r;
                    const bool ok = D.exact ? (st >= p.own_begin && st < p.own_end && st + p.m <= p.avail_len)
                                            : verify_exact_call(p, (long long)st) != 0;
                    if (ok) hm |= 1u << (4 * k + r);
                }
            }
    }
    else
    {
#pragma unroll
        for (int k = 0; k < 4; k++)
#pragma unroll
            for (int d = 0; d < 4; d++)
                if ((w[k] & p.fold) == p.K[d] && verify_exact_call(p, (long long)(unit + 4 * k) - d)) hm |= 1u << (4 * k);
    }
    return hm;
}

__device__ __noinline__ PartState count_tail(const CountDev &D, PartState S, uint64_t cov, uint64_t nl_lo, uint64_t nl_hi, bool window)
{
    const LitDevParams &p = D.p;
    const uint32_t lane = threadIdx.x & 31;
    if (p.avail_len < p.emit_len && cov >= nl_hi) return S;
    const uint64_t last_start = p.avail_len >= p.emit_len ? p.avail_len - p.emit_len : 0;
    uint64_t end = nl_hi > last_start + 1 ? nl_hi : last_start + 1;
    if (!window && end < cov + 1) end = cov + 1;
    for (uint64_t base = cov; base < end; base += 32)
    {
        settle(p, S, base > nl_lo ? base : nl_lo);
        const uint64_t q = base + lane;
        uint32_t hm = 0, nm = 0;
        if (q < end)
        {
            if (p.avail_len >= p.emit_len && q >= p.tail_start && q <= last_start && verify_exact(p, (long long)q)) hm = 1;
            if (!window && q == cov && p.avail_len >= p.emit_len)
                for (uint64_t s = p.tail_start; s < cov && s <= last_start; s++)
                    if (verify_exact(p, (long long)s)) hm = 1;
            if (q >= nl_lo && q < nl_hi && q < p.avail_len && p.text[q] == '\n') nm = 1;
            if (nm) hm = 0;
        }
        account(S, hm, nm);
        S.covered_to = base + 32;
    }
    return S;
}

#ifndef KREP_B200_COUNT_MINB
#define KREP_B200_COUNT_MINB 3
#endif
template <bool WINDOW, bool FOLD, bool MASKED>
__global__ void __launch_bounds__(256, KREP_B200_COUNT_MINB) k_count_lines(const __grid_constant__ CountDev D)
{
    const LitDevParams &p = D.p;
    const uint4 *__restrict__ t4 = reinterpret_cast<const uint4 *>(p.text);
    const uint32_t lane = threadIdx.x & 31;
    const uint32_t warp_global = (blockIdx.x * blockDim.x + threadIdx.x) >> 5, total_warps = (gridDim.x * blockDim.x) >> 5;
    const uint32_t k0 = p.K[0], k1 = p.K[1], k2 = p.K[2], k3 = p.K[3], fold = p.fold, mask = p.win_mask;
    const uint32_t c1 = p.mulc[0], c2 = p.mulc[1], c3 = p.mulc[2];
    for (uint32_t pi = warp_global; pi < D.n_parts; pi += total_warps)
    {
        const uint64_t ga = p.group_begin + (uint64_t)pi * D.part_groups;
        uint64_t gb = ga + D.part_groups;
        if (gb > p.group_end) gb = p.group_end;
        const bool last_part = pi + 1 == D.n_parts;
        const uint64_t nl_lo = ga * 16 > p.own_begin ? ga * 16 : p.own_begin;
        const uint64_t nl_hi = (last_part || gb * 16 > D.own_end) ? D.own_end : gb * 16;
        PartState S;
        S.covered_to = nl_lo;
        for (uint64_t g = ga; g < gb; g += 128)
        {
            uint4 v[4];
            uint32_t nx[4];
            bool ok[4];
#pragma unroll
            for (int u = 0; u < 4; u++)
            {
                const uint64_t gi = g + 32 * u + lane;
                ok[u] = gi < gb;
                v[u] = ok[u] ? ld_stream(t4 + gi) : make_uint4(0u, 0u, 0u, 0u);
                nx[u] = 0;
                if (WINDOW && ok[u] && (lane == 31 || gi + 1 >= gb)) nx[u] = __ldg(reinterpret_cast<const uint32_t *>(t4 + gi + 1));
            }
            uint32_t cand = 0;
#pragma unroll
            for (int u = 0; u < 4; u++)
            {
                bool h;
                if (WINDOW)
                {
                    const uint32_t nb = __shfl_down_sync(0xffffffffu, v[u].x, 1);
                    if (!(lane == 31 || g + 32 * u + lane + 1 >= gb)) nx[u] = nb;
                    h = hit_vec_w<FOLD, MASKED>(v[u], nx[u], fold, mask, k0, c1, c2, c3);
                }
                else
                    h = hit_vec<FOLD>(v[u], fold, k0, k1, k2, k3);
                cand |= (h && ok[u]) ? (1u << u) : 0u;
            }
            const uint32_t any = __reduce_or_sync(0xffffffffu, cand);
            if (any)
            {
                const uint64_t tile_lo = g * 16;
                settle(p, S, tile_lo > nl_lo ? tile_lo : nl_lo);
                const bool inside = tile_lo >= nl_lo && tile_lo + 2048 <= nl_hi;
                uint64_t st = pack_state(S);
#pragma unroll
                for (int u = 0; u < 4; u++)
                {
                    const uint64_t unit = tile_lo + 512ull * u + 16ull * lane;
                    uint32_t hm = 0, nm = 0;
                    if (ok[u])
                    {
                        if ((cand >> u) & 1u) hm = hit_mask16<WINDOW>(D, unit, v[u], nx[u]);
                        nm = nl_mask16(v[u]);
                        if (!inside) nm &= range_mask16(unit, nl_lo, nl_hi);
                    }
                    st = account_call(st, hm, nm);
                }
                unpack_state(st, S);
                S.covered_to = tile_lo + 2048;
            }
        }
        if (last_part && D.tail) S = count_tail(D, S, gb * 16, nl_lo, nl_hi, WINDOW);
        uint32_t flags = 0;
        if (S.has_hit)
        {
            if (S.pending && S.covered_to < nl_hi && scan_for_newline(p, S.covered_to, nl_hi)) S.pending = false;
            flags = LR_HAS_HIT | (S.first_open ? LR_FIRST_OPEN : 0u) | (S.pending ? LR_LAST_PENDING : 0u) | LR_HAS_NL;
        }
        else
        {
            const bool nl = S.seen_nl || (S.covered_to < nl_hi && scan_for_newline(p, S.covered_to, nl_hi));
            flags = nl ? LR_HAS_NL : 0u;
        }
        if (lane == 0) D.recs[pi] = LineRec{S.lines, flags};
    }
}

__host__ __device__ __forceinline__ void append_rec(uint64_t &lines, uint32_t &flags, uint64_t blines, uint32_t bflags)
{
    const bool ah = flags & LR_HAS_HIT, bh = bflags & LR_HAS_HIT;
    if (!bh)
    {
        if (ah && (bflags & LR_HAS_NL)) flags &= ~(uint32_t)LR_LAST_PENDING;
        flags |= bflags & LR_HAS_NL;
        return;
    }
    if (!ah)
    {
        const bool had_nl = flags & LR_HAS_NL;
        lines = blines;
        flags = bflags | LR_HAS_NL * had_nl;
        if (had_nl) flags &= ~(uint32_t)LR_FIRST_OPEN;
        return;
    }
    lines += blines;
    if ((flags & LR_LAST_PENDING) && (bflags & LR_FIRST_OPEN)) lines--;
    flags = LR_HAS_HIT | LR_HAS_NL | (flags & LR_FIRST_OPEN) | (bflags & LR_LAST_PENDING);
}

__global__ void __launch_bounds__(1024) k_count_finish(const LineRec *recs, uint32_t n, uint64_t *d_out, uint64_t *h_out)
{
    __shared__ uint64_t s_lines[1024];
    __shared__ uint32_t s_flags[1024];
    const uint32_t per = (n + blockDim.x - 1) / blockDim.x;
    const uint32_t a = threadIdx.x * per, b = a + per < n ? a + per : n;
    uint64_t lines = 0;
    uint32_t flags = 0;
    for (uint32_t i = a; i < b; i++) append_rec(lines, flags, recs[i].lines, recs[i].flags);
    s_lines[threadIdx.x] = lines;
    s_flags[threadIdx.x] = flags;
    __syncthreads();
    if (threadIdx.x == 0)
    {
        lines = 0;
        flags = 0;
        for (uint32_t t = 0; t < blockDim.x; t++) append_rec(lines, flags, s_lines[t], s_flags[t]);
        d_out[0] = lines;
        d_out[1] = flags;
        h_out[0] = lines;
        h_out[1] = flags;
    }
}

#define CKC(call)                                                                                  \
    do                                                                                             \
    {                                                                                              \
        cudaError_t e_ = (call);                                                                   \
        if (e_ != cudaSuccess)                                                                     \
        {                                                                                          \
            set_error(-2, "CUDA error %s at %s:%d (%s)", cudaGetErrorName(e_), __FILE__, __LINE__, \
                      cudaGetErrorString(e_));                                                     \
            return -2;                                                                             \
        }                                                                                          \
    } while (0)

bool count_lines_eligible(const Plan *plan, const search_params_t *P, int algo)
{
    if (!P->count_lines_mode || plan->is_ac || plan->is_regex || plan->emit_len != plan->m || plan->whole_word == 2) return false;
    if (plan->pattern.find('\n') != std::string::npos) return false;
    return algo == KREP_B200_ALGO_BMH || algo == KREP_B200_ALGO_KMP || algo == KREP_B200_ALGO_MEMCHR ||
           algo == KREP_B200_ALGO_MEMCHR_SHORT || algo == KREP_B200_ALGO_SSE42;
}

int ensure_line_out(DevCtx &E, uint64_t n)
{
    if (n <= E.line_out_cap) return 0;
    CKC(cudaDeviceSynchronize());
    cudaFree(E.d_line_out);
    cudaFreeHost(E.h_line_out);
    E.d_line_out = nullptr;
    E.h_line_out = nullptr;
    E.line_out_cap = 0;
    uint64_t cap = 64;
    while (cap < n) cap *= 2;
    CKC(cudaMalloc(&E.d_line_out, cap * 2 * sizeof(uint64_t)));
    CKC(cudaHostAlloc(&E.h_line_out, cap * 2 * sizeof(uint64_t), cudaHostAllocMapped | cudaHostAllocPortable));
    E.line_out_cap = cap;
    return 0;
}

int launch_count_lines(DevCtx &E, const Plan *plan, const krep_b200_shard_t *sh, cudaStream_t stream, uint64_t index)
{
    if (((uintptr_t)sh->d_text & 15) != 0)
    {
        set_error(-3, "shard text pointer must be 16-byte aligned");
        return -3;
    }
    const PlanDev *pd = plan_on_device(plan, E);
    if (!pd) return -2;
    if (ensure_line_out(E, index + 1) != 0) return -2;
    CountDev D;
    memset(&D, 0, sizeof D);
    LitDevParams &p = D.p;
    const uint64_t own_end = sh->own_end < sh->avail_len ? sh->own_end : sh->avail_len;
    p.text = (const uint8_t *)sh->d_text;
    p.avail_len = sh->avail_len;
    p.own_begin = sh->own_begin;
    p.own_end = own_end;
    p.global_offset = sh->global_offset;
    p.prev_byte = sh->prev_byte;
    p.next_byte = sh->next_byte;
    uint64_t total_groups;
    const bool window = plan->filter == FILTER_WINDOW4;
    if (!window)
    {
        total_groups = sh->avail_len / 16;
        p.tail_start = total_groups ? total_groups * 16 - 3 : 0;
    }
    else
    {
        total_groups = sh->avail_len >= 20 ? (sh->avail_len - 20) / 16 + 1 : 0;
        p.tail_start = total_groups * 16;
    }
    p.group_begin = sh->own_begin / 16;
    p.group_end = (own_end + 2) / 16 + 1;
    D.tail = p.group_end > total_groups ? 1u : 0u;
    if (p.group_end > total_groups) p.group_end = total_groups;
    if (p.group_begin > p.group_end) p.group_begin = p.group_end;
    p.m = plan->m;
    p.emit_len = plan->emit_len;
    for (int d = 0; d < 4; d++) p.K[d] = plan->K[d];
    p.fold = plan->fold;
    p.win_mask = plan->win_mask;
    p.mulc[0] = 1u << 24;
    p.mulc[1] = 1u << 16;
    p.mulc[2] = 1u << 8;
    p.pat_val = pd->d_pat_val;
    p.pat_mask = pd->d_pat_mask;
    p.whole_word = plan->whole_word;
    D.own_end = own_end;
    {
        bool letters = true;
        for (unsigned char ch : plan->pattern) letters &= is_alpha_c(ch);
        D.exact = (window && plan->m <= 4 && plan->whole_word == 0 && (plan->case_sensitive || letters)) ? 1u : 0u;
    }
    const uint64_t groups = p.group_end - p.group_begin;
    static uint32_t part_default = 0;
    if (!part_default)
    {
        const char *v = getenv("KREP_B200_COUNT_PART_KB");
        uint32_t kb_ = v && atoi(v) > 0 ? (uint32_t)atoi(v) : 64;
        part_default = std::max<uint32_t>(128, kb_ * 64 / 128 * 128);
    }
    uint64_t part = part_default;
    const uint64_t max_parts = 1u << 18;
    if ((groups + part - 1) / part > max_parts) part = ((groups + max_parts - 1) / max_parts + 127) / 128 * 128;
    D.part_groups = (uint32_t)part;
    D.n_parts = (uint32_t)std::max<uint64_t>((groups + part - 1) / part, 1);
    if (D.n_parts > E.line_recs_cap)
    {
        CKC(cudaStreamSynchronize(stream));
        cudaFree(E.d_line_recs);
        E.d_line_recs = nullptr;
        E.line_recs_cap = 0;
        const uint64_t cap = std::max<uint64_t>(D.n_parts, 1u << 16);
        CKC(cudaMalloc(&E.d_line_recs, cap * sizeof(LineRec)));
        E.line_recs_cap = cap;
    }
    D.recs = (LineRec *)E.d_line_recs;
    const bool folded = plan->fold != 0xFFFFFFFFu, masked = plan->win_mask != 0xFFFFFFFFu;
    const uint64_t want_blocks = ((uint64_t)D.n_parts + 7) / 8;
    const unsigned grid = (unsigned)std::min<uint64_t>(want_blocks, (uint64_t)E.sm_count * KREP_B200_COUNT_MINB);
    if (!window)
    {
        if (folded) k_count_lines<false, true, false><<<grid, 256, 0, stream>>>(D);
        else k_count_lines<false, false, false><<<grid, 256, 0, stream>>>(D);
    }
    else if (folded)
    {
        if (masked) k_count_lines<true, true, true><<<grid, 256, 0, stream>>>(D);
        else k_count_lines<true, true, false><<<grid, 256, 0, stream>>>(D);
    }
    else
    {
        if (masked) k_count_lines<true, false, true><<<grid, 256, 0, stream>>>(D);
        else k_count_lines<true, false, false><<<grid, 256, 0, stream>>>(D);
    }
    CKC(cudaGetLastError());
    k_count_finish<<<1, 1024, 0, stream>>>(D.recs, D.n_parts, E.d_line_out + 2 * index, E.h_line_out + 2 * index);
    CKC(cudaGetLastError());
    count_launch(2);
    return 0;
}

uint64_t combine_line_records(const uint64_t *recs, size_t n)
{
    uint64_t lines = 0;
    uint32_t flags = 0;
    for (size_t i = 0; i < n; i++) append_rec(lines, flags, recs[2 * i], (uint32_t)recs[2 * i + 1]);
    return lines;
}

}
```

### krep_b200/lib.py

```python
import ctypes as C
import os

from .abi import (CorpusSpec, DeviceResult, MatchResult, Params, SearchParams, Shard, SEARCH_FUNC, SIZE_MAX)

_HERE = os.path.dirname(os.path.abspath(__file__))
LIB_PATH = os.environ.get("KREP_B200_LIB") or os.path.join(_HERE, "libkrep_b200.so")

SEARCH_ENTRIES = {
    "boyer_moore": "krep_b200_boyer_moore_search",
    "kmp": "krep_b200_kmp_search",
    "memchr": "krep_b200_memchr_search",
    "memchr_short": "krep_b200_memchr_short_search",
    "sse42": "krep_b200_simd_sse42_search",
    "avx2": "krep_b200_simd_avx2_search",
    "avx512": "krep_b200_simd_avx512_search",
    "aho_corasick": "krep_b200_aho_corasick_search",
    "neon": "krep_b200_neon_search",
    "regex": "krep_b200_regex_search",
}

_lib = None


def load():
    global _lib
    if _lib is not None:
        return _lib
    if not os.path.exists(LIB_PATH):
        raise RuntimeError(f"{LIB_PATH} is missing: run `python -c 'import __graft_entry__ as g; g.build()'` "
                           "(there is no fallback implementation)")
    L = C.CDLL(LIB_PATH)
    sig = [C.POINTER(SearchParams), C.c_void_p, C.c_size_t, C.POINTER(MatchResult)]
    for name in SEARCH_ENTRIES.values():
        f = getattr(L, name)
        f.argtypes = sig
        f.restype = C.c_uint64
    L.krep_b200_init.argtypes = [C.c_int]
    L.krep_b200_init.restype = C.c_int
    L.krep_b200_last_error.restype = C.c_int
    L.krep_b200_last_error_string.restype = C.c_char_p
    L.krep_b200_version.restype = C.c_char_p
    L.krep_b200_set_only_matching.argtypes = [C.c_bool]
    L.krep_b200_get_only_matching.restype = C.c_bool
    L.krep_b200_set_force_no_simd.argtypes = [C.c_bool]
    L.krep_b200_set_algo_override.argtypes = [C.c_char_p]
    L.krep_b200_select_search_algorithm.argtypes = [C.POINTER(SearchParams)]
    L.krep_b200_select_search_algorithm.restype = C.c_void_p
    L.krep_b200_get_algorithm_name.argtypes = [C.c_void_p]
    L.krep_b200_get_algorithm_name.restype = C.c_char_p
    L.krep_b200_ac_trie_build.argtypes = [C.POINTER(SearchParams)]
    L.krep_b200_ac_trie_build.restype = C.c_void_p
    L.krep_b200_ac_trie_free.argtypes = [C.c_void_p]
    L.krep_b200_ac_trie_root_has_outputs.argtypes = [C.c_void_p]
    L.krep_b200_ac_trie_root_has_outputs.restype = C.c_bool
    L.krep_b200_match_result_init.argtypes = [C.c_uint64]
    L.krep_b200_match_result_init.restype = C.POINTER(MatchResult)
    L.krep_b200_match_result_add.argtypes = [C.POINTER(MatchResult), C.c_size_t, C.c_size_t]
    L.krep_b200_match_result_add.restype = C.c_bool
    L.krep_b200_match_result_free.argtypes = [C.POINTER(MatchResult)]
    L.krep_b200_match_result_merge.argtypes = [C.POINTER(MatchResult), C.POINTER(MatchResult), C.c_size_t]
    L.krep_b200_match_result_merge.restype = C.c_bool
    L.krep_b200_plan_create.argtypes = [C.POINTER(SearchParams), C.c_int]
    L.krep_b200_plan_create.restype = C.c_void_p
    L.krep_b200_plan_destroy.argtypes = [C.c_void_p]
    L.krep_b200_plan_filter_name.argtypes = [C.c_void_p]
    L.krep_b200_plan_filter_name.restype = C.c_char_p
    L.krep_b200_scan_shard.argtypes = [C.c_void_p, C.POINTER(Shard), C.c_int, C.c_void_p, C.POINTER(DeviceResult)]
    L.krep_b200_scan_shard.restype = C.c_int
    L.krep_b200_collect.argtypes = [C.c_void_p, C.POINTER(SearchParams), C.POINTER(DeviceResult), C.POINTER(MatchResult)]
    L.krep_b200_collect.restype = C.c_uint64
    L.krep_b200_replay.argtypes = [C.c_int, C.POINTER(SearchParams), C.c_bool, C.POINTER(C.c_uint64), C.c_uint64,
                                   C.c_void_p, C.c_size_t, C.POINTER(MatchResult)]
    L.krep_b200_replay.restype = C.c_uint64
    L.krep_b200_replay_lines.argtypes = [C.c_int, C.POINTER(SearchParams), C.c_bool, C.POINTER(C.c_uint64), C.c_uint64,
                                         C.POINTER(C.c_uint64), C.c_size_t, C.POINTER(MatchResult)]
    L.krep_b200_replay_lines.restype = C.c_uint64
    L.krep_b200_search_batch.argtypes = [C.c_void_p, C.POINTER(SearchParams), C.POINTER(C.c_char_p), C.POINTER(C.c_size_t), C.c_size_t,
                                         C.POINTER(C.c_uint64), C.POINTER(C.POINTER(MatchResult))]
    L.krep_b200_search_batch.restype = C.c_int
    L.krep_b200_scan_shard_begin.argtypes = [C.c_void_p, C.POINTER(Shard), C.c_int, C.c_void_p, C.POINTER(C.c_int)]
    L.krep_b200_scan_shard_begin.restype = C.c_int
    L.krep_b200_scan_shard_end.argtypes = [C.c_int, C.POINTER(DeviceResult)]
    L.krep_b200_scan_shard_end.restype = C.c_int
    L.krep_b200_export_packed.argtypes = [C.POINTER(DeviceResult), C.c_void_p, C.c_uint64, C.c_void_p]
    L.krep_b200_export_packed.restype = C.c_int
    L.krep_b200_export_packed_async.argtypes = [C.c_int, C.c_void_p, C.c_uint64]
    L.krep_b200_export_packed_async.restype = C.c_int
    L.krep_b200_merge_keys.argtypes = [C.POINTER(C.c_void_p), C.POINTER(C.c_uint64), C.c_uint32, C.c_void_p]
    L.krep_b200_merge_keys.restype = C.c_uint64
    L.krep_b200_set_devices.argtypes = [C.POINTER(C.c_int), C.c_int]
    L.krep_b200_device_count.restype = C.c_int
    L.krep_b200_search_shards.argtypes = [C.c_void_p, C.POINTER(SearchParams), C.POINTER(Shard), C.c_uint32, C.POINTER(MatchResult)]
    L.krep_b200_search_shards.restype = C.c_uint64
    L.krep_b200_export_keys.argtypes = [C.POINTER(DeviceResult), C.c_void_p, C.c_uint64, C.c_void_p]
    L.krep_b200_export_keys.restype = C.c_int
    L.krep_b200_regex_filter_host.argtypes = [C.POINTER(SearchParams), C.c_void_p, C.c_size_t, C.POINTER(C.c_uint64), C.c_uint64,
                                              C.POINTER(C.c_int)]
    L.krep_b200_regex_filter_host.restype = C.c_int64
    L.krep_b200_regex_count_mode.argtypes = [C.POINTER(SearchParams)]
    L.krep_b200_regex_count_mode.restype = C.c_int
    L.krep_b200_regex_count_host.argtypes = [C.POINTER(SearchParams), C.c_void_p, C.c_size_t, C.c_uint64]
    L.krep_b200_regex_count_host.restype = C.c_int64
    L.krep_b200_regex_match_mode.argtypes = [C.POINTER(SearchParams)]
    L.krep_b200_regex_match_mode.restype = C.c_int
    L.krep_b200_regex_matches_host.argtypes = [C.POINTER(SearchParams), C.c_void_p, C.c_size_t, C.c_uint64, C.POINTER(MatchResult)]
    L.krep_b200_regex_matches_host.restype = C.c_int64
    L.krep_b200_regex_scan_shard_raw.argtypes = [C.c_void_p, C.POINTER(Shard), C.c_int, C.POINTER(C.c_uint64), C.c_uint64,
                                                 C.POINTER(C.c_uint64)]
    L.krep_b200_regex_scan_shard_raw.restype = C.c_int64
    L.krep_b200_last_kernel_ms.restype = C.c_float
    L.krep_b200_launch_count.restype = C.c_uint64
    for n in ("krep_b200_ac_key_end", "krep_b200_ac_key_start"):
        getattr(L, n).argtypes = [C.c_uint64]
        getattr(L, n).restype = C.c_uint64
    L.krep_b200_ac_key_pattern.argtypes = [C.c_uint64]
    L.krep_b200_ac_key_pattern.restype = C.c_uint32
    L.krep_b200_corpus_generate.argtypes = [C.POINTER(CorpusSpec), C.c_void_p, C.c_uint64, C.c_uint64, C.c_void_p]
    L.krep_b200_corpus_generate.restype = C.c_int
    L.krep_b200_corpus_generate_host.argtypes = [C.POINTER(CorpusSpec), C.c_void_p, C.c_uint64, C.c_uint64]
    L.krep_b200_corpus_generate_host.restype = C.c_int
    _lib = L
    return L


def check(L=None):
    L = L or load()
    if L.krep_b200_last_error() != 0:
        raise RuntimeError("krep_b200: " + L.krep_b200_last_error_string().decode())


def search(func, params, text, with_result=True, text_ptr=None, text_len=None):
    L = load()
    L.krep_b200_set_only_matching(bool(params.only_matching))
    own_trie = False
    if func == "aho_corasick" and not params.struct.ac_trie:
        params.struct.ac_trie = L.krep_b200_ac_trie_build(params.ref())
        own_trie = True
    res = L.krep_b200_match_result_init(16) if with_result else None
    try:
        if text_ptr is None:
            buf = C.cast(C.c_char_p(text), C.c_void_p)
            n = len(text)
        else:
            buf, n = C.c_void_p(text_ptr), text_len
        cnt = getattr(L, SEARCH_ENTRIES[func])(params.ref(), buf, n, res)
        check(L)
        pos = []
        if res:
            r = res.contents
            pos = [(r.positions[i].start_offset, r.positions[i].end_offset) for i in range(r.count)]
        return int(cnt), pos
    finally:
        if res:
            L.krep_b200_match_result_free(res)
        if own_trie:
            L.krep_b200_ac_trie_free(params.struct.ac_trie)
            params.struct.ac_trie = None
        L.krep_b200_set_only_matching(False)


def make_spec(seed, plant_seed=0, plant_period=0, needle=b"", flags=0):
    s = CorpusSpec()
    s.seed = seed
    s.plant_seed = plant_seed
    s.plant_period = plant_period
    s._needle_keepalive = C.create_string_buffer(needle, max(len(needle), 1))
    s.needle = C.cast(s._needle_keepalive, C.c_char_p)
    s.needle_len = len(needle)
    s.flags = flags
    return s


def corpus_host(spec, offset, length):
    L = load()
    buf = C.create_string_buffer(length)
    rc = L.krep_b200_corpus_generate_host(C.byref(spec), buf, offset, length)
    if rc != 0:
        raise RuntimeError("corpus_generate_host failed")
    return buf.raw


def search_batch(func, params, texts, with_result=True):
    L = load()
    L.krep_b200_set_only_matching(bool(params.only_matching))
    own_trie = False
    if func == "aho_corasick" and not params.struct.ac_trie:
        params.struct.ac_trie = L.krep_b200_ac_trie_build(params.ref())
        own_trie = True
    n = len(texts)
    bufs = [C.create_string_buffer(t, max(len(t), 1)) for t in texts]
    tarr = (C.c_char_p * max(n, 1))(*[C.cast(b, C.c_char_p) for b in bufs])
    larr = (C.c_size_t * max(n, 1))(*[len(t) for t in texts])
    counts = (C.c_uint64 * max(n, 1))()
    res = [L.krep_b200_match_result_init(16) for _ in range(n)] if with_result else []
    rarr = (C.POINTER(MatchResult) * max(n, 1))(*res) if with_result else None
    try:
        entry = C.cast(getattr(L, SEARCH_ENTRIES[func]), C.c_void_p)
        rc = L.krep_b200_search_batch(entry, params.ref(), tarr, larr, n, counts, rarr)
        check(L)
        assert rc == 0, rc
        out = []
        for i in range(n):
            pos = []
            if with_result:
                r = res[i].contents
                pos = [(r.positions[k].start_offset, r.positions[k].end_offset) for k in range(r.count)]
            out.append((int(counts[i]), pos))
        return out
    finally:
        for r in res:
            L.krep_b200_match_result_free(r)
        if own_trie:
            L.krep_b200_ac_trie_free(params.struct.ac_trie)
            params.struct.ac_trie = None
        L.krep_b200_set_only_matching(False)
```

Before: 3120.

## Replace warp line-count state machine with carry-based fold and add host reference

Rewrites the per-warp line-count accounting for -c mode. The old branchy state machine (pending/covered_to, separate newline rescans, noinline verify calls) becomes a branch-light fold that derives line hits from carry propagation over ballot masks, with inlined hit-mask builders. It also factors out the setup code and adds a host-side implementation of the same partition counter, exposed through a new API call for checking results. The GPU path aims to cut divergence, call overhead and extra newline scans, at the cost of new carry arithmetic that must match the old semantics exactly.

New measurement: 3115 (median of 6 runs). No clear change (-0.2%).

```diff
diff --git a/include/krep_b200.h b/include/krep_b200.h
--- a/include/krep_b200.h
+++ b/include/krep_b200.h
@@ -171,6 +171,8 @@
 int krep_b200_count_lines_shard(const krep_b200_plan_t *plan, const search_params_t *params, const krep_b200_shard_t *shard,
                                 void *stream, krep_b200_line_count_t *out);
 uint64_t krep_b200_combine_line_counts(const krep_b200_line_count_t *recs, size_t n, size_t max_count);
+int krep_b200_count_lines_host(const search_params_t *params, int algo, const krep_b200_shard_t *shard, uint32_t part_kb,
+                               krep_b200_line_count_t *out);
 
 uint64_t krep_b200_collect(const krep_b200_plan_t *plan, const search_params_t *params,
                            const krep_b200_device_result_t *dev, match_result_t *result);
diff --git a/krep_b200/csrc/engine.h b/krep_b200/csrc/engine.h
--- a/krep_b200/csrc/engine.h
+++ b/krep_b200/csrc/engine.h
@@ -118,6 +118,7 @@
 bool count_lines_eligible(const Plan *plan, const search_params_t *P, int algo);
 int ensure_line_out(DevCtx &C, uint64_t n);
 int launch_count_lines(DevCtx &C, const Plan *plan, const krep_b200_shard_t *sh, cudaStream_t stream, uint64_t index);
+void count_lines_host(const Plan *plan, const krep_b200_shard_t *sh, uint32_t part_kb, uint64_t out[2]);
 uint64_t combine_line_records(const uint64_t *recs, size_t n);
 
 uint64_t merge_key_lists(const uint64_t *const *lists, const uint64_t *counts, uint32_t n_lists, uint64_t *dst);
diff --git a/krep_b200/csrc/host_api.cu b/krep_b200/csrc/host_api.cu
--- a/krep_b200/csrc/host_api.cu
+++ b/krep_b200/csrc/host_api.cu
@@ -1186,6 +1186,36 @@
     return 0;
 }
 
+int krep_b200_count_lines_host(const search_params_t *P, int algo, const krep_b200_shard_t *shard, uint32_t part_kb,
+                               krep_b200_line_count_t *out)
+{
+    std::lock_guard<std::recursive_mutex> lk(engine_mutex());
+    clear_error();
+    if (!P || !shard || !out)
+    {
+        set_error(-3, "krep_b200_count_lines_host: null argument");
+        return -3;
+    }
+    Plan *plan = plan_build(P, resolve_algo(P, algo), krep_b200_get_only_matching());
+    if (!plan) return -3;
+    int rc = 0;
+    if (!count_lines_eligible(plan, P, plan->algo))
+    {
+        set_error(-3, "krep_b200_count_lines_host: this plan's -c result needs the occurrence list");
+        rc = -3;
+    }
+    else
+    {
+        uint64_t rec[2];
+        count_lines_host(plan, shard, part_kb, rec);
+        out->lines = rec[0];
+        out->flags = (uint32_t)rec[1];
+        out->reserved = 0;
+    }
+    plan_free(plan);
+    return rc;
+}
+
 uint64_t krep_b200_combine_line_counts(const krep_b200_line_count_t *recs, size_t n, size_t max_count)
 {
     if (!recs) return 0;
diff --git a/krep_b200/csrc/lit_filters.cuh b/krep_b200/csrc/lit_filters.cuh
--- a/krep_b200/csrc/lit_filters.cuh
+++ b/krep_b200/csrc/lit_filters.cuh
@@ -3,12 +3,12 @@
 
 namespace kb {
 
-__device__ __forceinline__ bool dev_is_word(int c)
+__host__ __device__ __forceinline__ bool dev_is_word(int c)
 {
     return (c >= '0' && c <= '9') || (c >= 'A' && c <= 'Z') || (c >= 'a' && c <= 'z') || c == '_';
 }
 
-__device__ __forceinline__ unsigned verify_exact(const LitDevParams &p, long long cand)
+__host__ __device__ __forceinline__ unsigned verify_exact(const LitDevParams &p, long long cand)
 {
     if (cand < (long long)p.own_begin || cand >= (long long)p.own_end) return 0;
     const uint64_t c = (uint64_t)cand;
@@ -43,23 +43,32 @@
 }
 
 template <bool FOLD>
-__device__ __forceinline__ bool hit_word(uint32_t w, uint32_t fold, uint32_t k0, uint32_t k1, uint32_t k2, uint32_t k3)
+__host__ __device__ __forceinline__ bool hit_word(uint32_t w, uint32_t fold, uint32_t k0, uint32_t k1, uint32_t k2, uint32_t k3)
 {
     if (FOLD) w &= fold;
     return (w == k0) | (w == k1) | (w == k2) | (w == k3);
 }
 template <bool FOLD>
-__device__ __forceinline__ bool hit_vec(const uint4 &v, uint32_t fold, uint32_t k0, uint32_t k1, uint32_t k2, uint32_t k3)
+__host__ __device__ __forceinline__ bool hit_vec(const uint4 &v, uint32_t fold, uint32_t k0, uint32_t k1, uint32_t k2, uint32_t k3)
 {
     return hit_word<FOLD>(v.x, fold, k0, k1, k2, k3) | hit_word<FOLD>(v.y, fold, k0, k1, k2, k3) |
            hit_word<FOLD>(v.z, fold, k0, k1, k2, k3) | hit_word<FOLD>(v.w, fold, k0, k1, k2, k3);
 }
 
+__host__ __device__ __forceinline__ uint32_t umulhi32(uint32_t a, uint32_t b)
+{
+#ifdef __CUDA_ARCH__
+    return __umulhi(a, b);
+#else
+    return (uint32_t)(((uint64_t)a * b) >> 32);
+#endif
+}
+
 template <bool MASKED>
-__device__ __forceinline__ bool hit_pair(uint32_t lo, uint32_t hi, uint32_t mask, uint32_t k0, uint32_t c1, uint32_t c2,
+__host__ __device__ __forceinline__ bool hit_pair(uint32_t lo, uint32_t hi, uint32_t mask, uint32_t k0, uint32_t c1, uint32_t c2,
                                          uint32_t c3)
 {
-    uint32_t x0 = lo, x1 = hi * c1 + __umulhi(lo, c1), x2 = hi * c2 + __umulhi(lo, c2), x3 = hi * c3 + __umulhi(lo, c3);
+    uint32_t x0 = lo, x1 = hi * c1 + umulhi32(lo, c1), x2 = hi * c2 + umulhi32(lo, c2), x3 = hi * c3 + umulhi32(lo, c3);
     if (MASKED)
     {
         x0 &= mask; x1 &= mask; x2 &= mask; x3 &= mask;
@@ -67,7 +76,7 @@
     return (x0 == k0) | (x1 == k0) | (x2 == k0) | (x3 == k0);
 }
 template <bool FOLD, bool MASKED>
-__device__ __forceinline__ bool hit_vec_w(const uint4 &v, uint32_t nx, uint32_t fold, uint32_t mask, uint32_t k0,
+__host__ __device__ __forceinline__ bool hit_vec_w(const uint4 &v, uint32_t nx, uint32_t fold, uint32_t mask, uint32_t k0,
                                           uint32_t c1, uint32_t c2, uint32_t c3)
 {
     uint32_t w0 = v.x, w1 = v.y, w2 = v.z, w3 = v.w, w4 = nx;
diff --git a/krep_b200/csrc/scan_count.cu b/krep_b200/csrc/scan_count.cu
--- a/krep_b200/csrc/scan_count.cu
+++ b/krep_b200/csrc/scan_count.cu
@@ -1,8 +1,15 @@
 #include <algorithm>
+#include <string.h>
 #include "engine.h"
 #include "lit_filters.cuh"
 
 namespace kb {
+
+#ifdef __CUDA_ARCH__
+#define KB_UNROLL _Pragma("unroll")
+#else
+#define KB_UNROLL
+#endif
 
 enum : uint32_t
 {
@@ -21,32 +28,45 @@
 {
     LitDevParams p;
     uint64_t own_end;
+    uint64_t hit_end;
     uint32_t part_groups, n_parts;
     uint32_t exact;
     uint32_t tail;
     LineRec *recs;
 };
 
-struct PartState
+struct LineAcc
 {
     uint32_t lines = 0;
-    bool has_hit = false, first_open = false, pending = false, seen_nl = false;
-    uint64_t covered_to = 0;
+    bool open_hit = false;
+    bool has_hit = false, first_open = false, seen_nl = false;
 };
 
-__device__ __noinline__ unsigned verify_exact_call(const LitDevParams &p, long long cand) { return verify_exact(p, cand); }
-
-__device__ __forceinline__ uint32_t nl_nibble(uint32_t w)
+__host__ __device__ __forceinline__ uint32_t popc32(uint32_t x)
+{
+#ifdef __CUDA_ARCH__
+    return (uint32_t)__popc(x);
+#else
+    return (uint32_t)__builtin_popcount(x);
+#endif
+}
+
+__host__ __device__ __forceinline__ uint32_t nl_nibble(uint32_t w)
 {
     const uint32_t x = w ^ 0x0A0A0A0Au;
     const uint32_t y = ~(((x & 0x7F7F7F7Fu) + 0x7F7F7F7Fu) | x | 0x7F7F7F7Fu);
     return ((y >> 7) * 0x10204080u) >> 28;
 }
-__device__ __forceinline__ uint32_t nl_mask16(const uint4 &v)
+__host__ __device__ __forceinline__ uint32_t nl_mask16(const uint4 &v)
 {
     return nl_nibble(v.x) | (nl_nibble(v.y) << 4) | (nl_nibble(v.z) << 8) | (nl_nibble(v.w) << 12);
 }
-__device__ __forceinline__ uint32_t range_mask16(uint64_t unit, uint64_t lo, uint64_t hi)
+__host__ __device__ __forceinline__ uint32_t nl_any16(const uint4 &v)
+{
+    const uint32_t a = v.x ^ 0x0A0A0A0Au, b = v.y ^ 0x0A0A0A0Au, c = v.z ^ 0x0A0A0A0Au, d = v.w ^ 0x0A0A0A0Au;
+    return (((a - 0x01010101u) & ~a) | ((b - 0x01010101u) & ~b) | ((c - 0x01010101u) & ~c) | ((d - 0x01010101u) & ~d)) & 0x80808080u;
+}
+__host__ __device__ __forceinline__ uint32_t range_mask16(uint64_t unit, uint64_t lo, uint64_t hi)
 {
     uint32_t m = 0xFFFFu;
     if (unit < lo) m = lo - unit >= 16 ? 0u : (m & ~((1u << (uint32_t)(lo - unit)) - 1u));
@@ -54,186 +74,208 @@
     return m;
 }
 
-__device__ __noinline__ bool scan_for_newline(const LitDevParams &p, uint64_t lo, uint64_t hi)
-{
-    const uint32_t lane = threadIdx.x & 31;
-    if (hi > p.avail_len) hi = p.avail_len;
-    for (uint64_t base = lo & ~15ull; base < hi; base += 512)
-    {
-        const uint64_t unit = base + 16ull * lane;
-        uint32_t nm = 0;
-        if (unit < hi && unit + 16 > lo)
+struct LaneSum
+{
+    bool has_nl;
+    bool pre;
+    bool post;
+    uint32_t inner;
+};
+__host__ __device__ __forceinline__ LaneSum lane_summary(uint32_t hm, uint32_t nm)
+{
+    const uint32_t b = ~nm & 0xFFFFu, sum = hm + b, c = sum ^ hm ^ b;
+    const uint32_t segs = nm & c, first = segs & nm & (0u - nm);
+    const bool co = (sum >> 16) & 1u;
+    LaneSum s;
+    s.has_nl = nm != 0;
+    s.pre = s.has_nl ? first != 0 : co;
+    s.post = s.has_nl && co;
+    s.inner = popc32(segs) - (first != 0 ? 1u : 0u);
+    return s;
+}
+
+__host__ __device__ __forceinline__ void warp_fold(LineAcc &S, uint32_t A, uint32_t P, uint32_t Lm, uint32_t inner)
+{
+    const uint32_t X = P | (Lm << 1), b = ~A, a = X & b;
+    const uint64_t sum = (uint64_t)a + b + (S.open_hit ? 1u : 0u);
+    const uint32_t c = (uint32_t)sum ^ a ^ b;
+    if (!S.has_hit && !S.seen_nl && (X & (A ^ (A - 1u)))) S.first_open = true;
+    S.has_hit |= (P | Lm | inner) != 0;
+    S.seen_nl |= A != 0;
+    S.lines += popc32(A & (X | c)) + inner;
+    S.open_hit = ((sum >> 32) | (Lm >> 31)) & 1u;
+}
+
+__host__ __device__ __forceinline__ LineRec partition_record(const LineAcc &S)
+{
+    if (!S.has_hit) return LineRec{0u, S.seen_nl ? (uint32_t)LR_HAS_NL : 0u};
+    return LineRec{S.lines + (S.open_hit ? 1u : 0u),
+                   LR_HAS_HIT | LR_HAS_NL | (S.first_open ? LR_FIRST_OPEN : 0u) | (S.open_hit ? LR_LAST_PENDING : 0u)};
+}
+
+template <bool FOLD, bool MASKED>
+__host__ __device__ __forceinline__ uint32_t window_hits16(const uint4 &v, uint32_t nx, uint32_t fold, uint32_t mask, uint32_t k0)
+{
+    uint32_t w[5] = {v.x, v.y, v.z, v.w, nx};
+    if (FOLD)
+        KB_UNROLL for (int k = 0; k < 5; k++) w[k] &= fold;
+    uint32_t hm = 0;
+    KB_UNROLL for (int k = 0; k < 4; k++)
+    {
+        const uint32_t lo = w[k], hi = w[k + 1];
+        uint32_t x0 = lo, x1 = (lo >> 8) | (hi << 24), x2 = (lo >> 16) | (hi << 16), x3 = (lo >> 24) | (hi << 8);
+        if (MASKED)
         {
-            if (unit + 16 <= p.avail_len) nm = nl_mask16(__ldg(reinterpret_cast<const uint4 *>(p.text + unit)));
-            else
-                for (uint64_t q = unit; q < p.avail_len; q++) nm |= (p.text[q] == '\n' ? 1u : 0u) << (uint32_t)(q - unit);
-            nm &= range_mask16(unit, lo, hi);
+            x0 &= mask; x1 &= mask; x2 &= mask; x3 &= mask;
         }
-        if (__any_sync(0xffffffffu, nm != 0)) return true;
-    }
-    return false;
-}
-
-__device__ __forceinline__ void settle(const LitDevParams &p, PartState &S, uint64_t upto)
-{
-    if (S.covered_to < upto && (S.pending || (!S.has_hit && !S.seen_nl)))
-        if (scan_for_newline(p, S.covered_to, upto))
+        hm |= ((x0 == k0 ? 1u : 0u) | (x1 == k0 ? 2u : 0u) | (x2 == k0 ? 4u : 0u) | (x3 == k0 ? 8u : 0u)) << (4 * k);
+    }
+    return hm;
+}
+
+template <bool FOLD>
+__host__ __device__ __forceinline__ uint32_t aligned_cands16(const uint4 &v, uint32_t fold, uint32_t k0, uint32_t k1, uint32_t k2,
+                                                             uint32_t k3)
+{
+    const uint32_t w[4] = {v.x, v.y, v.z, v.w};
+    uint32_t cm = 0;
+    KB_UNROLL for (int k = 0; k < 4; k++)
+    {
+        const uint32_t x = FOLD ? w[k] & fold : w[k];
+        cm |= ((x == k0 ? 1u : 0u) | (x == k1 ? 2u : 0u) | (x == k2 ? 4u : 0u) | (x == k3 ? 8u : 0u)) << (4 * k);
+    }
+    return cm;
+}
+
+__host__ __device__ __forceinline__ uint32_t ctz32(uint32_t x)
+{
+#ifdef __CUDA_ARCH__
+    return (uint32_t)__ffs(x) - 1;
+#else
+    return (uint32_t)__builtin_ctz(x);
+#endif
+}
+
+template <bool WINDOW, bool FOLD, bool MASKED>
+__host__ __device__ __forceinline__ void lane_masks(const CountDev &D, uint64_t unit, const uint4 &v, uint32_t nx, bool cand,
+                                                    bool edge, uint64_t nl_lo, uint64_t nl_hi, uint32_t &hm, uint32_t &nm)
+{
+    const LitDevParams &p = D.p;
+    uint32_t cm = WINDOW ? window_hits16<FOLD, MASKED>(v, nx, p.fold, p.win_mask, p.K[0])
+                         : aligned_cands16<FOLD>(v, p.fold, p.K[0], p.K[1], p.K[2], p.K[3]);
+    if (!cand) cm = 0;
+    if (WINDOW && D.exact)
+    {
+        hm = cm;
+        if (edge) hm &= range_mask16(unit, p.own_begin, D.hit_end);
+    }
+    else
+    {
+        hm = 0;
+        while (cm)
         {
-            S.pending = false;
-            S.seen_nl = true;
+            const uint32_t b = ctz32(cm);
+            cm &= cm - 1;
+            const uint32_t pos = WINDOW ? b : b & ~3u;
+            if (verify_exact(p, (long long)(unit + pos) - (long long)(WINDOW ? 0u : b & 3u))) hm |= 1u << pos;
         }
-}
-
-__device__ __forceinline__ void account(PartState &S, uint32_t hm, uint32_t nm)
-{
-    const uint32_t lane = threadIdx.x & 31;
-    const bool has_nl = nm != 0;
-    const uint32_t fnl = has_nl ? (uint32_t)__ffs(nm) - 1 : 0, lnl = has_nl ? 31u - (uint32_t)__clz(nm) : 0;
-    const bool f = has_nl && (hm & ((1u << fnl) - 1u)) != 0;
-    const bool l = has_nl && ((hm >> lnl) >> 1) != 0;
-    uint32_t inner = 0;
-    if (__popc(nm) >= 2)
-    {
-        uint32_t prev = fnl, rest = nm & (nm - 1);
-        while (rest)
-        {
-            const uint32_t nx = (uint32_t)__ffs(rest) - 1;
-            if (hm & (((1u << nx) - 1u) & ~((2u << prev) - 1u))) inner++;
-            prev = nx;
-            rest &= rest - 1;
-        }
-    }
-    const uint32_t A = __ballot_sync(0xffffffffu, has_nl), T = __ballot_sync(0xffffffffu, !has_nl && hm != 0);
-    const uint32_t F = __ballot_sync(0xffffffffu, f), Lm = __ballot_sync(0xffffffffu, l);
-    uint32_t innersum = 0;
-    if (__ballot_sync(0xffffffffu, inner != 0)) innersum = __reduce_add_sync(0xffffffffu, inner);
-    if (A == 0)
-    {
-        if (T)
-        {
-            if (!S.pending)
-            {
-                S.lines++;
-                if (!S.has_hit && !S.seen_nl) S.first_open = true;
-            }
-            S.pending = true;
-            S.has_hit = true;
-        }
-        return;
-    }
-    const uint32_t j1 = (uint32_t)__ffs(A) - 1, jr = 31u - (uint32_t)__clz(A);
-    if ((T & ((1u << j1) - 1u)) || ((F >> j1) & 1u))
-    {
-        if (!S.pending)
-        {
-            S.lines++;
-            if (!S.has_hit && !S.seen_nl) S.first_open = true;
-        }
-        S.has_hit = true;
-    }
-    S.pending = false;
-    S.seen_nl = true;
-    bool gap = false;
-    if (has_nl && lane != j1)
-    {
-        const uint32_t below = A & ((1u << lane) - 1u);
-        const uint32_t pj = 31u - (uint32_t)__clz(below);
-        const uint32_t between = ((1u << lane) - 1u) & ~((2u << pj) - 1u);
-        gap = ((Lm >> pj) & 1u) || (T & between) || f;
-    }
-    const uint32_t G = __ballot_sync(0xffffffffu, gap);
-    S.lines += (uint32_t)__popc(G) + innersum;
-    if (G || innersum) S.has_hit = true;
-    if (((Lm >> jr) & 1u) || ((T >> jr) >> 1))
-    {
-        S.lines++;
-        S.has_hit = true;
-        S.pending = true;
-    }
-}
-
-__device__ __forceinline__ uint64_t pack_state(const PartState &S)
-{
-    return (uint64_t)S.lines | ((uint64_t)((S.has_hit ? 1u : 0u) | (S.first_open ? 2u : 0u) | (S.pending ? 4u : 0u) | (S.seen_nl ? 8u : 0u)) << 32);
-}
-__device__ __forceinline__ void unpack_state(uint64_t k, PartState &S)
-{
-    S.lines = (uint32_t)k;
-    const uint32_t f = (uint32_t)(k >> 32);
-    S.has_hit = f & 1u;
-    S.first_open = f & 2u;
-    S.pending = f & 4u;
-    S.seen_nl = f & 8u;
-}
-__device__ __noinline__ uint64_t account_call(uint64_t packed, uint32_t hm, uint32_t nm)
-{
-    PartState S;
-    unpack_state(packed, S);
-    account(S, hm, nm);
-    return pack_state(S);
-}
-
-template <bool WINDOW>
-__device__ __noinline__ uint32_t hit_mask16(const CountDev &D, uint64_t unit, const uint4 &v, uint32_t nx)
-{
-    const LitDevParams &p = D.p;
-    const uint32_t w[5] = {v.x, v.y, v.z, v.w, nx};
-    uint32_t hm = 0;
-    if (WINDOW)
-    {
-        const uint32_t mask = p.fold & p.win_mask, k0 = p.K[0];
-#pragma unroll
-        for (int k = 0; k < 4; k++)
-#pragma unroll
-            for (int r = 0; r < 4; r++)
-            {
-                const uint32_t win = r == 0 ? w[k] : __funnelshift_r(w[k], w[k + 1], 8 * r);
-                if ((win & mask) == k0)
-                {
-                    const uint64_t st = unit + 4 * k + r;
-                    const bool ok = D.exact ? (st >= p.own_begin && st < p.own_end && st + p.m <= p.avail_len)
-                                            : verify_exact_call(p, (long long)st) != 0;
-                    if (ok) hm |= 1u << (4 * k + r);
-                }
-            }
-    }
-    else
-    {
-#pragma unroll
-        for (int k = 0; k < 4; k++)
-#pragma unroll
-            for (int d = 0; d < 4; d++)
-                if ((w[k] & p.fold) == p.K[d] && verify_exact_call(p, (long long)(unit + 4 * k) - d)) hm |= 1u << (4 * k);
-    }
-    return hm;
-}
-
-__device__ __noinline__ PartState count_tail(const CountDev &D, PartState S, uint64_t cov, uint64_t nl_lo, uint64_t nl_hi, bool window)
-{
-    const LitDevParams &p = D.p;
-    const uint32_t lane = threadIdx.x & 31;
-    if (p.avail_len < p.emit_len && cov >= nl_hi) return S;
+    }
+    nm = nl_mask16(v);
+    if (edge) nm &= range_mask16(unit, nl_lo, nl_hi);
+}
+
+struct PartGeom
+{
+    uint64_t ga, gb, nl_lo, nl_hi;
+    bool last;
+};
+__host__ __device__ __forceinline__ bool edge_tile(const CountDev &D, const PartGeom &G, uint64_t tile_lo)
+{
+    return tile_lo < G.nl_lo || tile_lo + 2048 > G.nl_hi || tile_lo + 2048 > D.hit_end;
+}
+__host__ __device__ __forceinline__ PartGeom part_geom(const CountDev &D, uint32_t pi)
+{
+    PartGeom G;
+    G.ga = D.p.group_begin + (uint64_t)pi * D.part_groups;
+    G.gb = G.ga + D.part_groups;
+    if (G.gb > D.p.group_end) G.gb = D.p.group_end;
+    G.last = pi + 1 == D.n_parts;
+    G.nl_lo = G.ga * 16 > D.p.own_begin ? G.ga * 16 : D.p.own_begin;
+    G.nl_hi = (G.last || G.gb * 16 > D.own_end) ? D.own_end : G.gb * 16;
+    return G;
+}
+
+__host__ __device__ __forceinline__ bool has_newline(const uint4 &v, uint64_t unit, bool edge, const PartGeom &G)
+{
+    return (edge ? nl_mask16(v) & range_mask16(unit, G.nl_lo, G.nl_hi) : nl_any16(v)) != 0;
+}
+
+__host__ __device__ __forceinline__ uint64_t tail_end(const LitDevParams &p, uint64_t cov, uint64_t nl_hi, bool window)
+{
+    if (p.avail_len < p.emit_len && cov >= nl_hi) return cov;
     const uint64_t last_start = p.avail_len >= p.emit_len ? p.avail_len - p.emit_len : 0;
     uint64_t end = nl_hi > last_start + 1 ? nl_hi : last_start + 1;
     if (!window && end < cov + 1) end = cov + 1;
+    return end;
+}
+__host__ __device__ __forceinline__ void tail_masks(const LitDevParams &p, uint64_t q, uint64_t cov, uint64_t end, uint64_t nl_lo,
+                                                    uint64_t nl_hi, bool window, uint32_t &hm, uint32_t &nm)
+{
+    hm = nm = 0;
+    if (q >= end) return;
+    const uint64_t last_start = p.avail_len >= p.emit_len ? p.avail_len - p.emit_len : 0;
+    if (p.avail_len >= p.emit_len && q >= p.tail_start && q <= last_start && verify_exact(p, (long long)q)) hm = 1;
+    if (!window && q == cov && p.avail_len >= p.emit_len)
+        for (uint64_t s = p.tail_start; s < cov && s <= last_start; s++)
+            if (verify_exact(p, (long long)s)) hm = 1;
+    if (q >= nl_lo && q < nl_hi && q < p.avail_len && p.text[q] == '\n') nm = 1;
+    if (nm) hm = 0;
+}
+
+__device__ __forceinline__ void fold_lanes(LineAcc &S, uint32_t hm, uint32_t nm)
+{
+    const LaneSum s = lane_summary(hm, nm);
+    warp_fold(S, __ballot_sync(0xffffffffu, s.has_nl), __ballot_sync(0xffffffffu, s.pre), __ballot_sync(0xffffffffu, s.post),
+              __reduce_add_sync(0xffffffffu, s.inner));
+}
+
+__device__ __noinline__ LineAcc count_tail(const CountDev &D, LineAcc S, uint64_t cov, uint64_t nl_lo, uint64_t nl_hi, bool window)
+{
+    const uint32_t lane = threadIdx.x & 31;
+    const uint64_t end = tail_end(D.p, cov, nl_hi, window);
     for (uint64_t base = cov; base < end; base += 32)
     {
-        settle(p, S, base > nl_lo ? base : nl_lo);
-        const uint64_t q = base + lane;
-        uint32_t hm = 0, nm = 0;
-        if (q < end)
-        {
-            if (p.avail_len >= p.emit_len && q >= p.tail_start && q <= last_start && verify_exact(p, (long long)q)) hm = 1;
-            if (!window && q == cov && p.avail_len >= p.emit_len)
-                for (uint64_t s = p.tail_start; s < cov && s <= last_start; s++)
-                    if (verify_exact(p, (long long)s)) hm = 1;
-            if (q >= nl_lo && q < nl_hi && q < p.avail_len && p.text[q] == '\n') nm = 1;
-            if (nm) hm = 0;
-        }
-        account(S, hm, nm);
-        S.covered_to = base + 32;
+        uint32_t hm, nm;
+        tail_masks(D.p, base + lane, cov, end, nl_lo, nl_hi, window, hm, nm);
+        fold_lanes(S, hm, nm);
     }
     return S;
+}
+
+template <bool WINDOW>
+__device__ __forceinline__ void load_tile(const uint4 *__restrict__ t4, uint64_t g, uint64_t gb, uint32_t lane, uint4 (&v)[4],
+                                          uint32_t &nx_end)
+{
+#pragma unroll
+    for (int u = 0; u < 4; u++)
+    {
+        const uint64_t gi = g + 32 * u + lane;
+        v[u] = gi < gb ? ld_stream(t4 + gi) : make_uint4(0u, 0u, 0u, 0u);
+    }
+    nx_end = 0;
+    if (WINDOW && lane == 31 && g + 127 < gb) nx_end = __ldg(reinterpret_cast<const uint32_t *>(t4 + g + 128));
+}
+
+template <bool WINDOW>
+__device__ __forceinline__ uint32_t next_word(const uint4 *__restrict__ t4, const uint4 (&v)[4], uint32_t nx_end, int u, uint64_t g,
+                                              uint64_t gb, uint32_t lane)
+{
+    const uint32_t nb = __shfl_sync(0xffffffffu, u < 3 ? v[u < 3 ? u + 1 : 0].x : 0u, 0);
+    uint32_t nx = __shfl_down_sync(0xffffffffu, v[u].x, 1);
+    if (lane == 31) nx = u < 3 ? nb : nx_end;
+    const uint64_t gi = g + 32 * u + lane;
+    if (gi < gb && gi + 1 >= gb) nx = __ldg(reinterpret_cast<const uint32_t *>(t4 + gi + 1));
+    return nx;
 }
 
 #ifndef KREP_B200_COUNT_MINB
@@ -250,81 +292,160 @@
     const uint32_t c1 = p.mulc[0], c2 = p.mulc[1], c3 = p.mulc[2];
     for (uint32_t pi = warp_global; pi < D.n_parts; pi += total_warps)
     {
-        const uint64_t ga = p.group_begin + (uint64_t)pi * D.part_groups;
-        uint64_t gb = ga + D.part_groups;
-        if (gb > p.group_end) gb = p.group_end;
-        const bool last_part = pi + 1 == D.n_parts;
-        const uint64_t nl_lo = ga * 16 > p.own_begin ? ga * 16 : p.own_begin;
-        const uint64_t nl_hi = (last_part || gb * 16 > D.own_end) ? D.own_end : gb * 16;
-        PartState S;
-        S.covered_to = nl_lo;
-        for (uint64_t g = ga; g < gb; g += 128)
+        const PartGeom G = part_geom(D, pi);
+        LineAcc S;
+        uint4 v[4];
+        uint32_t nx_end;
+        load_tile<WINDOW>(t4, G.ga, G.gb, lane, v, nx_end);
+        for (uint64_t g = G.ga; g < G.gb; g += 128)
         {
-            uint4 v[4];
-            uint32_t nx[4];
-            bool ok[4];
-#pragma unroll
-            for (int u = 0; u < 4; u++)
-            {
-                const uint64_t gi = g + 32 * u + lane;
-                ok[u] = gi < gb;
-                v[u] = ok[u] ? ld_stream(t4 + gi) : make_uint4(0u, 0u, 0u, 0u);
-                nx[u] = 0;
-                if (WINDOW && ok[u] && (lane == 31 || gi + 1 >= gb)) nx[u] = __ldg(reinterpret_cast<const uint32_t *>(t4 + gi + 1));
-            }
+            uint4 vn[4];
+            uint32_t nxn_end;
+            load_tile<WINDOW>(t4, g + 128, G.gb, lane, vn, nxn_end);
             uint32_t cand = 0;
 #pragma unroll
             for (int u = 0; u < 4; u++)
             {
                 bool h;
                 if (WINDOW)
-                {
-                    const uint32_t nb = __shfl_down_sync(0xffffffffu, v[u].x, 1);
-                    if (!(lane == 31 || g + 32 * u + lane + 1 >= gb)) nx[u] = nb;
-                    h = hit_vec_w<FOLD, MASKED>(v[u], nx[u], fold, mask, k0, c1, c2, c3);
-                }
+                    h = hit_vec_w<FOLD, MASKED>(v[u], next_word<WINDOW>(t4, v, nx_end, u, g, G.gb, lane), fold, mask, k0, c1, c2, c3);
                 else
                     h = hit_vec<FOLD>(v[u], fold, k0, k1, k2, k3);
-                cand |= (h && ok[u]) ? (1u << u) : 0u;
+                cand |= (h && g + 32 * u + lane < G.gb) ? (1u << u) : 0u;
             }
+            const uint64_t tile_lo = g * 16;
+            const bool edge = edge_tile(D, G, tile_lo);
             const uint32_t any = __reduce_or_sync(0xffffffffu, cand);
             if (any)
             {
-                const uint64_t tile_lo = g * 16;
-                settle(p, S, tile_lo > nl_lo ? tile_lo : nl_lo);
-                const bool inside = tile_lo >= nl_lo && tile_lo + 2048 <= nl_hi;
-                uint64_t st = pack_state(S);
 #pragma unroll
                 for (int u = 0; u < 4; u++)
                 {
                     const uint64_t unit = tile_lo + 512ull * u + 16ull * lane;
-                    uint32_t hm = 0, nm = 0;
-                    if (ok[u])
+                    if ((any >> u) & 1u)
                     {
-                        if ((cand >> u) & 1u) hm = hit_mask16<WINDOW>(D, unit, v[u], nx[u]);
-                        nm = nl_mask16(v[u]);
-                        if (!inside) nm &= range_mask16(unit, nl_lo, nl_hi);
+                        uint32_t hm, nm;
+                        const uint32_t nx = WINDOW ? next_word<WINDOW>(t4, v, nx_end, u, g, G.gb, lane) : 0u;
+                        lane_masks<WINDOW, FOLD, MASKED>(D, unit, v[u], nx, (cand >> u) & 1u, edge, G.nl_lo, G.nl_hi, hm, nm);
+                        fold_lanes(S, hm, nm);
                     }
-                    st = account_call(st, hm, nm);
+                    else if (S.open_hit || !S.seen_nl)
+                    {
+                        if (__any_sync(0xffffffffu, has_newline(v[u], unit, edge, G))) warp_fold(S, 1u, 0u, 0u, 0u);
+                    }
                 }
-                unpack_state(st, S);
-                S.covered_to = tile_lo + 2048;
+            }
+            else if (S.open_hit || !S.seen_nl)
+            {
+                bool nl = false;
+#pragma unroll
+                for (int u = 0; u < 4; u++) nl |= has_newline(v[u], tile_lo + 512ull * u + 16ull * lane, edge, G);
+                if (__any_sync(0xffffffffu, nl)) warp_fold(S, 1u, 0u, 0u, 0u);
+            }
+#pragma unroll
+            for (int u = 0; u < 4; u++) v[u] = vn[u];
+            nx_end = nxn_end;
+        }
+        if (G.last && D.tail) S = count_tail(D, S, G.gb * 16, G.nl_lo, G.nl_hi, WINDOW);
+        if (lane == 0) D.recs[pi] = partition_record(S);
+    }
+}
+
+template <bool WINDOW, bool FOLD, bool MASKED>
+static LineRec count_partition_host(const CountDev &D, uint32_t pi)
+{
+    const LitDevParams &p = D.p;
+    const PartGeom G = part_geom(D, pi);
+    LineAcc S;
+    for (uint64_t g = G.ga; g < G.gb; g += 128)
+    {
+        uint4 v[4][32];
+        uint32_t nx[4][32], cand[32] = {0}, any = 0;
+        for (int u = 0; u < 4; u++)
+            for (uint32_t lane = 0; lane < 32; lane++)
+            {
+                const uint64_t gi = g + 32 * u + lane;
+                v[u][lane] = make_uint4(0u, 0u, 0u, 0u);
+                if (gi < G.gb) memcpy(&v[u][lane], p.text + 16 * gi, 16);
+            }
+        for (int u = 0; u < 4; u++)
+            for (uint32_t lane = 0; lane < 32; lane++)
+            {
+                const uint64_t gi = g + 32 * u + lane;
+                const bool ok = gi < G.gb;
+                nx[u][lane] = 0;
+                bool h;
+                if (WINDOW)
+                {
+                    if (ok && (lane == 31 || gi + 1 >= G.gb)) memcpy(&nx[u][lane], p.text + 16 * (gi + 1), 4);
+                    else if (ok) nx[u][lane] = v[u][lane + 1].x;
+                    h = hit_vec_w<FOLD, MASKED>(v[u][lane], nx[u][lane], p.fold, p.win_mask, p.K[0], p.mulc[0], p.mulc[1], p.mulc[2]);
+                }
+                else
+                    h = hit_vec<FOLD>(v[u][lane], p.fold, p.K[0], p.K[1], p.K[2], p.K[3]);
+                cand[lane] |= (h && ok) ? (1u << u) : 0u;
+                any |= cand[lane];
+            }
+        const uint64_t tile_lo = g * 16;
+        const bool edge = edge_tile(D, G, tile_lo);
+        if (any)
+        {
+            for (int u = 0; u < 4; u++)
+            {
+                bool vec_cand = false, nl = false;
+                for (uint32_t lane = 0; lane < 32; lane++)
+                {
+                    vec_cand |= (cand[lane] >> u) & 1u;
+                    nl |= has_newline(v[u][lane], tile_lo + 512ull * u + 16ull * lane, edge, G);
+                }
+                if (!vec_cand)
+                {
+                    if ((S.open_hit || !S.seen_nl) && nl) warp_fold(S, 1u, 0u, 0u, 0u);
+                    continue;
+                }
+                uint32_t A = 0, P = 0, Lm = 0, inner = 0;
+                for (uint32_t lane = 0; lane < 32; lane++)
+                {
+                    uint32_t hm, nm;
+                    lane_masks<WINDOW, FOLD, MASKED>(D, tile_lo + 512ull * u + 16ull * lane, v[u][lane], nx[u][lane],
+                                                     (cand[lane] >> u) & 1u, edge, G.nl_lo, G.nl_hi, hm, nm);
+                    const LaneSum s = lane_summary(hm, nm);
+                    A |= (s.has_nl ? 1u : 0u) << lane;
+                    P |= (s.pre ? 1u : 0u) << lane;
+                    Lm |= (s.post ? 1u : 0u) << lane;
+                    inner += s.inner;
+                }
+                warp_fold(S, A, P, Lm, inner);
             }
         }
-        if (last_part && D.tail) S = count_tail(D, S, gb * 16, nl_lo, nl_hi, WINDOW);
-        uint32_t flags = 0;
-        if (S.has_hit)
+        else if (S.open_hit || !S.seen_nl)
         {
-            if (S.pending && S.covered_to < nl_hi && scan_for_newline(p, S.covered_to, nl_hi)) S.pending = false;
-            flags = LR_HAS_HIT | (S.first_open ? LR_FIRST_OPEN : 0u) | (S.pending ? LR_LAST_PENDING : 0u) | LR_HAS_NL;
+            bool nl = false;
+            for (int u = 0; u < 4; u++)
+                for (uint32_t lane = 0; lane < 32; lane++) nl |= has_newline(v[u][lane], tile_lo + 512ull * u + 16ull * lane, edge, G);
+            if (nl) warp_fold(S, 1u, 0u, 0u, 0u);
         }
-        else
+    }
+    if (G.last && D.tail)
+    {
+        const uint64_t cov = G.gb * 16, end = tail_end(p, cov, G.nl_hi, WINDOW);
+        for (uint64_t base = cov; base < end; base += 32)
         {
-            const bool nl = S.seen_nl || (S.covered_to < nl_hi && scan_for_newline(p, S.covered_to, nl_hi));
-            flags = nl ? LR_HAS_NL : 0u;
+            uint32_t A = 0, P = 0, Lm = 0, inner = 0;
+            for (uint32_t lane = 0; lane < 32; lane++)
+            {
+                uint32_t hm, nm;
+                tail_masks(p, base + lane, cov, end, G.nl_lo, G.nl_hi, WINDOW, hm, nm);
+                const LaneSum s = lane_summary(hm, nm);
+                A |= (s.has_nl ? 1u : 0u) << lane;
+                P |= (s.pre ? 1u : 0u) << lane;
+                Lm |= (s.post ? 1u : 0u) << lane;
+                inner += s.inner;
+            }
+            warp_fold(S, A, P, Lm, inner);
         }
-        if (lane == 0) D.recs[pi] = LineRec{S.lines, flags};
-    }
+    }
+    return partition_record(S);
 }
 
 __host__ __device__ __forceinline__ void append_rec(uint64_t &lines, uint32_t &flags, uint64_t blines, uint32_t bflags)
@@ -410,17 +531,8 @@
     return 0;
 }
 
-int launch_count_lines(DevCtx &E, const Plan *plan, const krep_b200_shard_t *sh, cudaStream_t stream, uint64_t index)
-{
-    if (((uintptr_t)sh->d_text & 15) != 0)
-    {
-        set_error(-3, "shard text pointer must be 16-byte aligned");
-        return -3;
-    }
-    const PlanDev *pd = plan_on_device(plan, E);
-    if (!pd) return -2;
-    if (ensure_line_out(E, index + 1) != 0) return -2;
-    CountDev D;
+static void count_setup(const Plan *plan, const krep_b200_shard_t *sh, uint32_t part_kb, CountDev &D)
+{
     memset(&D, 0, sizeof D);
     LitDevParams &p = D.p;
     const uint64_t own_end = sh->own_end < sh->avail_len ? sh->own_end : sh->avail_len;
@@ -456,8 +568,6 @@
     p.mulc[0] = 1u << 24;
     p.mulc[1] = 1u << 16;
     p.mulc[2] = 1u << 8;
-    p.pat_val = pd->d_pat_val;
-    p.pat_mask = pd->d_pat_mask;
     p.whole_word = plan->whole_word;
     D.own_end = own_end;
     {
@@ -465,19 +575,34 @@
         for (unsigned char ch : plan->pattern) letters &= is_alpha_c(ch);
         D.exact = (window && plan->m <= 4 && plan->whole_word == 0 && (plan->case_sensitive || letters)) ? 1u : 0u;
     }
+    D.hit_end = !D.exact ? ~0ull : std::min<uint64_t>(own_end, sh->avail_len >= plan->m ? sh->avail_len - plan->m + 1 : 0);
     const uint64_t groups = p.group_end - p.group_begin;
-    static uint32_t part_default = 0;
-    if (!part_default)
+    if (!part_kb)
     {
         const char *v = getenv("KREP_B200_COUNT_PART_KB");
-        uint32_t kb_ = v && atoi(v) > 0 ? (uint32_t)atoi(v) : 64;
-        part_default = std::max<uint32_t>(128, kb_ * 64 / 128 * 128);
-    }
-    uint64_t part = part_default;
+        part_kb = v && atoi(v) > 0 ? (uint32_t)atoi(v) : 64;
+    }
+    uint64_t part = std::max<uint64_t>(128, (uint64_t)part_kb * 64 / 128 * 128);
     const uint64_t max_parts = 1u << 18;
     if ((groups + part - 1) / part > max_parts) part = ((groups + max_parts - 1) / max_parts + 127) / 128 * 128;
     D.part_groups = (uint32_t)part;
     D.n_parts = (uint32_t)std::max<uint64_t>((groups + part - 1) / part, 1);
+}
+
+int launch_count_lines(DevCtx &E, const Plan *plan, const krep_b200_shard_t *sh, cudaStream_t stream, uint64_t index)
+{
+    if (((uintptr_t)sh->d_text & 15) != 0)
+    {
+        set_error(-3, "shard text pointer must be 16-byte aligned");
+        return -3;
+    }
+    const PlanDev *pd = plan_on_device(plan, E);
+    if (!pd) return -2;
+    if (ensure_line_out(E, index + 1) != 0) return -2;
+    CountDev D;
+    count_setup(plan, sh, 0, D);
+    D.p.pat_val = pd->d_pat_val;
+    D.p.pat_mask = pd->d_pat_mask;
     if (D.n_parts > E.line_recs_cap)
     {
         CKC(cudaStreamSynchronize(stream));
@@ -489,6 +614,7 @@
         E.line_recs_cap = cap;
     }
     D.recs = (LineRec *)E.d_line_recs;
+    const bool window = plan->filter == FILTER_WINDOW4;
     const bool folded = plan->fold != 0xFFFFFFFFu, masked = plan->win_mask != 0xFFFFFFFFu;
     const uint64_t want_blocks = ((uint64_t)D.n_parts + 7) / 8;
     const unsigned grid = (unsigned)std::min<uint64_t>(want_blocks, (uint64_t)E.sm_count * KREP_B200_COUNT_MINB);
@@ -514,6 +640,28 @@
     return 0;
 }
 
+void count_lines_host(const Plan *plan, const krep_b200_shard_t *sh, uint32_t part_kb, uint64_t out[2])
+{
+    CountDev D;
+    count_setup(plan, sh, part_kb, D);
+    D.p.pat_val = plan->h_val.data();
+    D.p.pat_mask = plan->h_msk.data();
+    const bool window = plan->filter == FILTER_WINDOW4;
+    const bool folded = plan->fold != 0xFFFFFFFFu, masked = plan->win_mask != 0xFFFFFFFFu;
+    uint64_t lines = 0;
+    uint32_t flags = 0;
+    for (uint32_t pi = 0; pi < D.n_parts; pi++)
+    {
+        LineRec r;
+        if (!window) r = folded ? count_partition_host<false, true, false>(D, pi) : count_partition_host<false, false, false>(D, pi);
+        else if (folded) r = masked ? count_partition_host<true, true, true>(D, pi) : count_partition_host<true, true, false>(D, pi);
+        else r = masked ? count_partition_host<true, false, true>(D, pi) : count_partition_host<true, false, false>(D, pi);
+        append_rec(lines, flags, r.lines, r.flags);
+    }
+    out[0] = lines;
+    out[1] = flags;
+}
+
 uint64_t combine_line_records(const uint64_t *recs, size_t n)
 {
     uint64_t lines = 0;
diff --git a/krep_b200/lib.py b/krep_b200/lib.py
--- a/krep_b200/lib.py
+++ b/krep_b200/lib.py
@@ -97,6 +97,8 @@
     L.krep_b200_regex_filter_host.argtypes = [C.POINTER(SearchParams), C.c_void_p, C.c_size_t, C.POINTER(C.c_uint64), C.c_uint64,
                                               C.POINTER(C.c_int)]
     L.krep_b200_regex_filter_host.restype = C.c_int64
+    L.krep_b200_count_lines_host.argtypes = [C.POINTER(SearchParams), C.c_int, C.POINTER(Shard), C.c_uint32, C.c_void_p]
+    L.krep_b200_count_lines_host.restype = C.c_int
     L.krep_b200_regex_count_mode.argtypes = [C.POINTER(SearchParams)]
     L.krep_b200_regex_count_mode.restype = C.c_int
     L.krep_b200_regex_count_host.argtypes = [C.POINTER(SearchParams), C.c_void_p, C.c_size_t, C.c_uint64]
```
